# mbitsnbites/himg

Hardware: AMD Instinct MI355X
Metric: Mpixels/s encode+decode, 4K RGBA q=50 (higher is better)
Workload: dtype u8/i16/i32 integer

## Files before the change

himg_amd/__init__.py:

```python
import ctypes as C
import os

import numpy as np

from .build import LIB, build_lib

HIMG_OK = 0
HIMG_ERR_ARG = -1
HIMG_ERR_HIP = -2
HIMG_ERR_UNSUPPORTED = -3
HIMG_ERR_FORMAT = -4
HIMG_ERR_CAPACITY = -5
HIMG_ERR_TARGET = -6

HIMG_DT_F32 = 0
HIMG_DT_F16 = 1
HIMG_DT_BF16 = 2

SYNTH = {"grad": 0, "gradn": 1, "rand": 2, "randtile": 3}

DBG = {
    "avg": 0, "lowres": 1, "lres_sym": 2, "fres_sym": 3, "lres_hist": 4, "fres_hist": 5,
    "lres_len": 6, "fres_len": 7, "lres_code": 8, "fres_code": 9, "fres_row_bytes": 10,
    "dec_stats": 11, "parse_stats": 12, "rowcount_stats": 13, "loop_counts": 14, "fres_tok_sym": 15, "tok_cnt": 16,
}
DBG_DECODER = 0x100

_lib = None


class HimgError(RuntimeError):
    def __init__(self, code, msg=""):
        super().__init__("himg_hip error %d %s" % (code, msg))
        self.code = code


def lib():
    global _lib
    if _lib is not None:
        return _lib
    path = LIB
    if not os.path.exists(path):
        path = build_lib()
    try:
        import torch
    except ImportError:
        pass
    L = C.CDLL(path)
    vp, i32, u32, u64, sz = C.c_void_p, C.c_int, C.c_uint32, C.c_uint64, C.c_size_t
    P = C.POINTER
    L.himg_hip_create.argtypes = [i32, P(vp)]
    L.himg_hip_destroy.argtypes = [vp]
    L.himg_hip_destroy.restype = None
    L.himg_hip_last_error.argtypes = [vp]
    L.himg_hip_last_error.restype = C.c_char_p
    L.himg_hip_max_packed_size.argtypes = [i32, i32, i32]
    L.himg_hip_max_packed_size.restype = sz
    L.himg_hip_tok_layout.argtypes = [i32, i32, i32, i32, i32, i32, P(i32)]
    L.himg_hip_encode.argtypes = [vp, vp, i32, i32, i32, i32, i32, i32, P(vp), P(sz)]
    L.himg_hip_decode.argtypes = [vp, vp, sz, P(vp), P(i32), P(i32), P(i32)]
    L.himg_hip_encode_to.argtypes = [vp, vp, i32, i32, i32, i32, i32, i32, vp, sz, P(sz)]
    L.himg_hip_decode_to.argtypes = [vp, vp, sz, vp, sz, P(i32), P(i32), P(i32)]
    L.himg_hip_fetch_last.argtypes = [vp, vp, sz, P(sz)]
    L.himg_hip_peek.argtypes = [vp, sz, P(i32), P(i32), P(i32)]
    L.himg_hip_set_option.argtypes = [vp, i32, i32]
    L.himg_hip_get_option.argtypes = [vp, i32, C.POINTER(C.c_int)]
    L.himg_hip_encode_batch.argtypes = [vp, vp, i32, i32, i32, i32, i32, i32, i32, vp, vp, vp]
    L.himg_hip_decode_batch.argtypes = [vp, vp, vp, i32, vp, vp, vp, vp, vp]
    L.himg_hip_free.argtypes = [vp]
    L.himg_hip_free.restype = None
    L.himg_hip_host_alloc.argtypes = [sz]
    L.himg_hip_host_alloc.restype = vp
    L.himg_hip_host_free.argtypes = [vp]
    L.himg_hip_host_free.restype = None
    L.himg_hip_encode_device.argtypes = [vp, vp, i32, i32, i32, i32, i32, i32, i32, vp, sz, vp, vp, vp]
    L.himg_hip_decode_device.argtypes = [vp, vp, sz, vp, i32, i32, i32, i32, vp, vp, vp]
    L.himg_hip_encode_device_q.argtypes = [vp, vp, i32, i32, i32, i32, i32, vp, i32, vp, sz, vp, vp, vp]
    L.himg_hip_windows_extent.argtypes = [vp, i32, i32, vp, i32, i32, P(sz)]
    L.himg_hip_encode_windows_device.argtypes = [vp, vp, vp, i32, i32, vp, i32, i32, vp, i32, vp, sz, vp, vp, vp]
    L.himg_hip_encode_window_to.argtypes = [vp, vp, vp, i32, i32, i32, i32, i32, i32, i32, vp, sz, P(sz)]
    L.himg_hip_encode_sizes_device.argtypes = [vp, vp, i32, i32, i32, i32, i32, vp, i32, vp, vp, vp]
    L.himg_hip_budget_probes.argtypes = [i32, i32]
    L.himg_hip_encode_budget_device.argtypes = [vp, vp, i32, i32, i32, i32, i32, i32, i32, i32, vp, vp, sz, vp, vp, vp, vp]
    L.himg_hip_encode_budget_to.argtypes = [vp, vp, i32, i32, i32, i32, i32, i32, i32, sz, vp, sz, P(sz), P(i32)]
    L.himg_hip_encode_budget_batch.argtypes = [vp, vp, i32, i32, i32, i32, i32, i32, i32, i32, vp, vp, vp, vp, vp]
    L.himg_hip_encode_sse_device.argtypes = [vp, vp, i32, i32, i32, i32, i32, vp, i32, vp, vp, vp]
    L.himg_hip_encode_target_device.argtypes = [vp, vp, i32, i32, i32, i32, i32, i32, i32, i32, vp, vp, sz, vp, vp, vp, vp, vp]
    L.himg_hip_encode_target_to.argtypes = [vp, vp, i32, i32, i32, i32, i32, i32, i32, u64, vp, sz, P(sz), P(i32), P(u64)]
    L.himg_hip_encode_target_batch.argtypes = [vp, vp, i32, i32, i32, i32, i32, i32, i32, i32, vp, vp, vp, vp, vp, vp]
    L.himg_hip_psnr_to_sse.argtypes = [C.c_double, i32, i32, i32, P(u64)]
    L.himg_hip_decode_rows_device.argtypes = [vp, vp, C.c_uint32, i32, i32, i32, i32, i32, vp, vp, vp]
    L.himg_hip_decode_index_device.argtypes = [vp, vp, C.c_uint32, i32, i32, i32, vp, vp, vp, vp]
    L.himg_hip_decode_rows_indexed_device.argtypes = [vp, vp, C.c_uint32, i32, i32, i32, i32, i32, vp, vp, vp, vp]
    L.himg_hip_decode_rows_after_head_device.argtypes = [vp, vp, C.c_uint32, i32, i32, i32, i32, i32, vp, vp, vp, vp]
    L.himg_hip_decode_head_device.argtypes = [vp, vp, C.c_uint32, i32, i32, i32, vp]
    L.himg_hip_decode_first_device.argtypes = [vp, vp, C.c_uint32, i32, i32, i32, vp, vp, vp]
    L.himg_hip_decode_walk_device.argtypes = [vp, vp, C.c_uint32, i32, i32, i32, vp, vp, vp, vp]
    L.himg_hip_decode_walk_wait.argtypes = [vp]
    L.himg_hip_decode_walk_ranges_device.argtypes = [vp, vp, C.c_uint32, i32, i32, i32, C.POINTER(C.c_int), i32, vp, vp, vp, vp]
    L.himg_hip_decode_walk_wait_range.argtypes = [vp, i32]
    L.himg_hip_index_host.argtypes = [vp, sz, i32, P(i32), P(i32), P(i32), vp, sz, P(C.c_uint32)]
    L.himg_hip_preview_peek.argtypes = [vp, sz, sz, P(i32), P(i32), P(i32), P(sz)]
    L.himg_hip_region_peek.argtypes = [vp, sz, i32, i32, i32, i32, i32, vp]
    L.himg_hip_decode_region_to.argtypes = [vp, vp, sz, i32, i32, i32, i32, vp, sz, P(i32), P(i32), P(i32)]
    L.himg_hip_decode_region_device.argtypes = [vp, vp, sz, vp, i32, i32, i32, i32, i32, i32, i32, i32, vp, vp, vp]
    L.himg_hip_decode_regions_device.argtypes = [vp, vp, sz, vp, i32, i32, i32, i32, vp, i32, i32, vp, vp, vp]
    L.himg_hip_tensor_bytes.argtypes = [vp, i32, i32, i32, P(sz)]
    L.himg_hip_decode_tensor_device.argtypes = [vp, vp, sz, vp, i32, i32, i32, i32, vp, vp, vp, vp]
    L.himg_hip_decode_regions_tensor_device.argtypes = [vp, vp, sz, vp, i32, i32, i32, i32, vp, i32, i32, vp, vp, vp, vp]
    L.himg_hip_dst_extent.argtypes = [vp, i32, i32, vp, i32, i32, P(sz)]
    L.himg_hip_decode_into_device.argtypes = [vp, vp, sz, vp, i32, i32, i32, i32, vp, vp, vp, vp, vp]
    L.himg_hip_decode_regions_into_device.argtypes = [vp, vp, sz, vp, i32, i32, i32, i32, vp, i32, i32, vp, vp, vp, vp, vp]
    L.himg_hip_decode_into_to.argtypes = [vp, vp, sz, vp, vp, i32, i32, P(i32), P(i32), P(i32)]
    L.himg_hip_decode_regions_batch.argtypes = [vp, vp, vp, i32, vp, vp, vp, vp, vp, vp]
    L.himg_hip_scaled_size.argtypes = [i32, i32, i32, P(i32), P(i32)]
    L.himg_hip_decode_scaled_device.argtypes = [vp, vp, sz, vp, i32, i32, i32, i32, i32, vp, vp, vp]
    L.himg_hip_decode_scaled_to.argtypes = [vp, vp, sz, i32, vp, sz, P(i32), P(i32), P(i32)]
    L.himg_hip_decode_scaled_batch.argtypes = [vp, vp, vp, i32, i32, vp, vp, vp, vp, vp]
    L.himg_hip_pyramid_size.argtypes = [i32, i32, i32, P(i32), P(i32)]
    L.himg_hip_decode_pyramid_device.argtypes = [vp, vp, sz, vp, i32, i32, i32, i32, vp, vp, vp]
    L.himg_hip_decode_pyramid_to.argtypes = [vp, vp, sz, vp, vp, P(i32), P(i32), P(i32)]
    L.himg_hip_scaled_region_peek.argtypes = [vp, sz, i32, i32, i32, i32, i32, i32, vp]
    L.himg_hip_decode_scaled_region_to.argtypes = [vp, vp, sz, i32, i32, i32, i32, i32, vp, sz, P(i32), P(i32), P(i32)]
    L.himg_hip_decode_scaled_regions_device.argtypes = [vp, vp, sz, vp, i32, i32, i32, i32, i32, vp, i32, i32, vp, vp, vp]
    L.himg_hip_decode_scaled_regions_batch.argtypes = [vp, vp, vp, i32, i32, vp, vp, vp, vp, vp, vp]
    L.himg_hip_preview_to.argtypes = [vp, vp, sz, vp, sz, P(i32), P(i32), P(i32)]
    L.himg_hip_preview_batch.argtypes = [vp, vp, vp, i32, vp, vp, vp, vp, vp]
    L.himg_hip_preview_device.argtypes = [vp, vp, sz, vp, i32, i32, i32, i32, vp, vp, vp]
    L.himg_hip_prefix_peek.argtypes = [vp, sz, i32, vp]
    L.himg_hip_decode_prefix_to.argtypes = [vp, vp, sz, vp, sz, P(i32), P(i32), P(i32), P(i32)]
    L.himg_hip_decode_prefix_device.argtypes = [vp, vp, sz, vp, i32, i32, i32, i32, vp, vp, vp, vp]
    L.himg_hip_create_multi.argtypes = [vp, i32, P(vp)]
    L.himg_hip_destroy_multi.argtypes = [vp]
    L.himg_hip_destroy_multi.restype = None
    L.himg_hip_multi_count.argtypes = [vp]
    L.himg_hip_multi_last_error.argtypes = [vp]
    L.himg_hip_multi_last_error.restype = C.c_char_p
    L.himg_hip_multi_set_option.argtypes = [vp, i32, i32]
    L.himg_hip_multi_encode_batch.argtypes = [vp, vp, i32, i32, i32, i32, i32, i32, i32, vp, vp, vp]
    L.himg_hip_multi_decode_batch.argtypes = [vp, vp, vp, i32, vp, vp, vp, vp, vp]
    L.himg_hip_multi_encode.argtypes = [vp, vp, i32, i32, i32, i32, i32, i32, P(vp), P(sz)]
    L.himg_hip_multi_decode.argtypes = [vp, vp, sz, P(vp), P(i32), P(i32), P(i32)]
    L.himg_hip_shard_stats.argtypes = [vp, vp, i32, i32, i32, i32, i32, i32, i32, i32, vp, vp, vp]
    L.himg_hip_shard_row_bits.argtypes = [vp, vp, vp, vp]
    L.himg_hip_shard_emit.argtypes = [vp, vp, vp, sz, vp, vp]
    L.himg_hip_shard_assemble.argtypes = [vp, vp, vp, vp, sz, vp, sz, vp, vp, vp]
    L.himg_hip_shard_head.argtypes = [vp, vp, vp, vp, sz, vp, vp, vp, vp]
    L.himg_hip_shard_finish.argtypes = [vp, vp, sz, vp, vp]
    L.himg_hip_debug_read.argtypes = [vp, i32, i32, vp, sz, P(sz)]
    L.himg_hip_profile_enable.argtypes = [vp, i32]
    L.himg_hip_profile_reset.argtypes = [vp]
    L.himg_hip_profile_read.argtypes = [vp, P(i32), P(C.c_char_p), P(C.c_double), P(i32)]
    L.himg_synth_fill.argtypes = [i32, u64, i32, i32, vp]
    L.himg_fnv1a64.argtypes = [vp, sz]
    L.himg_fnv1a64.restype = u64
    L.himg_tables_shift.argtypes = [i32, i32, vp]
    L.himg_tables_shift.restype = None
    L.himg_tables_lowres_map.argtypes = [i32, vp]
    L.himg_tables_lowres_map.restype = None
    L.himg_tables_fullres_map.argtypes = [vp]
    L.himg_tables_fullres_map.restype = None
    L.himg_tables_map_to_8bit.argtypes = [vp, i32]
    L.himg_tables_map_to_8bit.restype = C.c_uint8
    _lib = L
    return L



def synth(kind, seed, width, height):
    a = np.empty((height, width, 4), np.uint8)
    rc = lib().himg_synth_fill(SYNTH[kind], seed, width, height, a.ctypes.data)
    if rc:
        raise HimgError(rc, "synth")
    return a


def fnv1a64(buf):
    b = np.ascontiguousarray(np.frombuffer(buf, np.uint8) if isinstance(buf, (bytes, bytearray)) else buf)
    return "%016x" % lib().himg_fnv1a64(b.ctypes.data, b.nbytes)


def max_packed_size(width, height, channels):
    return int(lib().himg_hip_max_packed_size(width, height, channels))


def budget_probes(qmin=0, qmax=100):
    n = lib().himg_hip_budget_probes(int(qmin), int(qmax))
    if n < 0:
        raise HimgError(n, "budget_probes")
    return n


def psnr_to_sse(psnr_db, width, height, channels):
    v = C.c_uint64()
    rc = lib().himg_hip_psnr_to_sse(float(psnr_db), int(width), int(height), int(channels), C.byref(v))
    if rc:
        raise HimgError(rc, "psnr_to_sse")
    return v.value


def tok_layout(width, height, channels=4, pixel_stride=None, row_tokens=-1, batch=1):
    out = (C.c_int32 * 6)()
    rc = lib().himg_hip_tok_layout(width, height, pixel_stride or channels, channels, row_tokens, batch, out)
    if rc != 0:
        raise ValueError("himg_hip_tok_layout: %d" % rc)
    return {"seg": out[0], "nseg": out[1], "cap": out[2], "stage_need": out[3], "stage": out[4], "tokens": bool(out[5])}


def pinned_empty(nbytes):
    import weakref
    ptr = lib().himg_hip_host_alloc(int(nbytes))
    if not ptr:
        raise MemoryError("himg_hip_host_alloc(%d)" % nbytes)
    buf = (C.c_uint8 * int(nbytes)).from_address(ptr)
    weakref.finalize(buf, lib().himg_hip_host_free, ptr)
    return np.frombuffer(buf, np.uint8)


def psnr(a, b):
    d = a.astype(np.float64) - b.astype(np.float64)
    mse = float(np.mean(d * d))
    return float("inf") if mse == 0 else 10.0 * np.log10(255.0 * 255.0 / mse)



_OPTIONS = {"fix_t2": 1, "count_wave": 2, "emit_rows": 3, "row_tokens": 4, "front": 5}


class Engine:

    def __init__(self, device=0):
        self._ctx = C.c_void_p()
        rc = lib().himg_hip_create(device, C.byref(self._ctx))
        if rc:
            raise HimgError(rc, "himg_hip_create (no usable GPU? there is no CPU fallback)")
        self.device = device
        self.fix_t2 = bool(self.get_option("fix_t2"))

    def close(self):
        if self._ctx:
            lib().himg_hip_destroy(self._ctx)
            self._ctx = C.c_void_p()

    def __del__(self):
        try:
            self.close()
        except Exception:
            pass

    def _check(self, rc, what):
        if rc:
            raise HimgError(rc, "%s: %s" % (what, lib().himg_hip_last_error(self._ctx).decode()))

    def _batch(self, fn, what, streams, outs, frame_bytes, *mid):
        n = len(streams)
        if outs is None:
            outs = [np.empty(max(frame_bytes(i, s_) or 0, 1), np.uint8) for i, s_ in enumerate(streams)]
        src = (C.c_void_p * n)(*[s_.ctypes.data for s_ in streams])
        szs = (C.c_size_t * n)(*[s_.nbytes for s_ in streams])
        dst = (C.c_void_p * n)(*[o.ctypes.data for o in outs])
        caps = (C.c_size_t * n)(*[o.nbytes for o in outs])
        ws, hs, cs = (C.c_int * n)(), (C.c_int * n)(), (C.c_int * n)()
        self._check(fn(self._ctx, src, szs, n, *mid, dst, caps, ws, hs, cs), what)
        return [o.ravel()[: ws[i] * hs[i] * cs[i]].reshape(hs[i], ws[i], cs[i]) for i, o in enumerate(outs)]

    def _encode_to(self, fn, what, img, channels, pixel_stride, mid, **results):
        img = np.ascontiguousarray(img, np.uint8)
        h, w, ch, stride = _image_geom(img, channels, pixel_stride)
        n = C.c_size_t()
        rc = fn(self._ctx, img.ctypes.data, w, h, stride, ch, *mid, None, 0, C.byref(n),
                *[C.byref(v) for v in results.values()])
        if rc != HIMG_ERR_CAPACITY or n.value == 0:
            e = HimgError(rc if rc != HIMG_OK else HIMG_ERR_ARG,
                          "%s: %s" % (what, lib().himg_hip_last_error(self._ctx).decode()))
            for name, v in results.items():
                setattr(e, name, v.value)
            raise e
        out = np.empty(n.value, np.uint8)
        self._check(lib().himg_hip_fetch_last(self._ctx, out.ctypes.data, out.nbytes, C.byref(n)), what)
        return (out, *[v.value for v in results.values()])

    def _encode_batch(self, fn, what, frames, outs, mid, results=(), soft=()):
        frames = [np.ascontiguousarray(f, np.uint8) for f in frames]
        n = len(frames)
        h, w, ch, stride = _image_geom(frames[0])
        if outs is None:
            outs = [np.empty(max_packed_size(w, h, ch), np.uint8) for _ in range(n)]
        src = (C.c_void_p * n)(*[f.ctypes.data for f in frames])
        dst = (C.c_void_p * n)(*[o.ctypes.data for o in outs])
        caps = (C.c_size_t * n)(*[o.nbytes for o in outs])
        sizes = (C.c_size_t * n)()
        rc = fn(self._ctx, src, n, w, h, stride, ch, *mid, dst, caps, sizes, *results)
        if rc not in (HIMG_OK, *soft):
            self._check(rc, what)
        return [o[: sizes[i]] for i, o in enumerate(outs)], rc

    def encode(self, img, quality=50, use_ycbcr=True, channels=None, pixel_stride=None):
        return self._encode_to(lib().himg_hip_encode_to, "encode", img, channels, pixel_stride,
                               (quality, 1 if use_ycbcr else 0))[0]

    def encode_window(self, data, src, x, y, w, h, quality=50, use_ycbcr=True, channels=None):
        data = _as_u8(data)
        ch = src.pixel_stride if channels is None else channels
        n = C.c_size_t()
        rc = lib().himg_hip_encode_window_to(self._ctx, data.ctypes.data, C.byref(src), ch, int(x), int(y), int(w),
                                             int(h), quality, 1 if use_ycbcr else 0, None, 0, C.byref(n))
        if rc != HIMG_ERR_CAPACITY or n.value == 0:
            self._check(rc if rc != HIMG_OK else HIMG_ERR_ARG, "encode_window")
        out = np.empty(n.value, np.uint8)
# ... 284 lines not shown
                                                         C.c_void_p(stream))
        self._check(rc, "decode_scaled_regions_device")

    def get_option(self, option):
        opt = _OPTIONS[option] if isinstance(option, str) else int(option)
        v = C.c_int(0)
        self._check(lib().himg_hip_get_option(self._ctx, opt, C.byref(v)), "get_option")
        return v.value

    def set_option(self, option, value):
        opt = _OPTIONS[option] if isinstance(option, str) else int(option)
        self._check(lib().himg_hip_set_option(self._ctx, opt, int(value)), "set_option")
        if opt == 1:
            self.fix_t2 = bool(value)

    def encode_device(self, d_frames, batch, width, height, pixel_stride, channels, quality,
                      use_ycbcr, d_out, out_stride, d_sizes, d_status, stream=0):
        rc = lib().himg_hip_encode_device(self._ctx, _ptr(d_frames), batch, width, height,
                                          pixel_stride, channels, quality, 1 if use_ycbcr else 0,
                                          _ptr(d_out), out_stride, _ptr(d_sizes), _ptr(d_status),
                                          C.c_void_p(stream))
        self._check(rc, "encode_device")

    def encode_device_q(self, d_frames, batch, width, height, pixel_stride, channels, qualities,
                        use_ycbcr, d_out, out_stride, d_sizes, d_status, stream=0):
        q = np.ascontiguousarray(np.asarray(qualities, np.int32).reshape(batch))
        rc = lib().himg_hip_encode_device_q(self._ctx, _ptr(d_frames), batch, width, height, pixel_stride, channels,
                                            q.ctypes.data, 1 if use_ycbcr else 0, _ptr(d_out), out_stride,
                                            _ptr(d_sizes), _ptr(d_status), C.c_void_p(stream))
        self._check(rc, "encode_device_q")

    def encode_windows_device(self, d_src, src, batch, channels, origins, w, h, qualities, use_ycbcr, d_out,
                              out_stride, d_sizes, d_status, stream=0):
        q = np.ascontiguousarray(np.asarray(qualities, np.int32).reshape(batch))
        org = np.ascontiguousarray(np.asarray(origins, np.int32).reshape(batch, 2))
        rc = lib().himg_hip_encode_windows_device(self._ctx, _ptr(d_src), C.byref(src), batch, channels,
                                                  org.ctypes.data, int(w), int(h), q.ctypes.data,
                                                  1 if use_ycbcr else 0, _ptr(d_out), out_stride, _ptr(d_sizes),
                                                  _ptr(d_status), C.c_void_p(stream))
        self._check(rc, "encode_windows_device")

    def encode_sizes_device(self, d_frames, batch, width, height, pixel_stride, channels, qualities,
                            use_ycbcr, d_sizes, d_status, stream=0):
        q = np.ascontiguousarray(np.asarray(qualities, np.int32).reshape(batch))
        rc = lib().himg_hip_encode_sizes_device(self._ctx, _ptr(d_frames), batch, width, height, pixel_stride,
                                                channels, q.ctypes.data, 1 if use_ycbcr else 0, _ptr(d_sizes),
                                                _ptr(d_status), C.c_void_p(stream))
        self._check(rc, "encode_sizes_device")

    def encode_budget_device(self, d_frames, batch, width, height, pixel_stride, channels, qmin, qmax,
                             use_ycbcr, budgets, d_out, out_stride, d_sizes, d_quality, d_status, stream=0):
        b = np.ascontiguousarray(np.minimum(np.asarray(budgets, np.uint64), 0xffffffff).astype(np.uint32).reshape(batch))
        rc = lib().himg_hip_encode_budget_device(self._ctx, _ptr(d_frames), batch, width, height, pixel_stride,
                                                 channels, int(qmin), int(qmax), 1 if use_ycbcr else 0,
                                                 b.ctypes.data, _ptr(d_out), out_stride, _ptr(d_sizes),
                                                 _ptr(d_quality), _ptr(d_status), C.c_void_p(stream))
        self._check(rc, "encode_budget_device")

    def encode_sse_device(self, d_frames, batch, width, height, pixel_stride, channels, qualities,
                          use_ycbcr, d_sse, d_status, stream=0):
        q = np.ascontiguousarray(np.asarray(qualities, np.int32).reshape(batch))
        rc = lib().himg_hip_encode_sse_device(self._ctx, _ptr(d_frames), batch, width, height, pixel_stride,
                                              channels, q.ctypes.data, 1 if use_ycbcr else 0, _ptr(d_sse),
                                              _ptr(d_status), C.c_void_p(stream))
        self._check(rc, "encode_sse_device")

    def encode_target_device(self, d_frames, batch, width, height, pixel_stride, channels, qmin, qmax,
                             use_ycbcr, max_sses, d_out, out_stride, d_sizes, d_quality, d_sse, d_status, stream=0):
        t = np.ascontiguousarray(np.array([min(max(int(x), 0), 2 ** 64 - 1) for x in max_sses], np.uint64).reshape(batch))
        rc = lib().himg_hip_encode_target_device(self._ctx, _ptr(d_frames), batch, width, height, pixel_stride,
                                                 channels, int(qmin), int(qmax), 1 if use_ycbcr else 0,
                                                 t.ctypes.data, _ptr(d_out), out_stride, _ptr(d_sizes),
                                                 _ptr(d_quality), _ptr(d_sse), _ptr(d_status), C.c_void_p(stream))
        self._check(rc, "encode_target_device")

    def decode_device(self, d_packed, in_stride, h_sizes, batch, width, height, channels, d_out,
                      d_status, stream=0):
        hs = np.ascontiguousarray(h_sizes, np.uint32)
        rc = lib().himg_hip_decode_device(self._ctx, _ptr(d_packed), in_stride, hs.ctypes.data,
                                          batch, width, height, channels, _ptr(d_out),
                                          _ptr(d_status), C.c_void_p(stream))
        self._check(rc, "decode_device")

    def decode_tensor_device(self, d_packed, in_stride, h_sizes, batch, width, height, channels, desc, d_out,
                             d_status, stream=0):
        hs = np.ascontiguousarray(h_sizes, np.uint32)
        rc = lib().himg_hip_decode_tensor_device(self._ctx, _ptr(d_packed), in_stride, hs.ctypes.data,
                                                 batch, width, height, channels, C.byref(desc), _ptr(d_out),
                                                 _ptr(d_status), C.c_void_p(stream))
        self._check(rc, "decode_tensor_device")

    def decode_rows_device(self, d_packed, packed_size, width, height, channels, row0, row1,
                           d_out_rows, d_status, stream=0):
        rc = lib().himg_hip_decode_rows_device(self._ctx, _ptr(d_packed), int(packed_size), width,
                                               height, channels, row0, row1, _ptr(d_out_rows),
                                               _ptr(d_status), C.c_void_p(stream))
        self._check(rc, "decode_rows_device")

    def decode_index_device(self, d_packed, packed_size, width, height, channels, d_row_index,
                            d_rows_first, d_status, stream=0):
        rc = lib().himg_hip_decode_index_device(self._ctx, _ptr(d_packed), int(packed_size), width, height,
                                                channels, _ptr(d_row_index), _ptr(d_rows_first),
                                                _ptr(d_status), C.c_void_p(stream))
        self._check(rc, "decode_index_device")

    def decode_rows_indexed_device(self, d_packed, packed_size, width, height, channels, row0, row1,
                                   d_row_index, d_out_rows, d_status, stream=0):
        rc = lib().himg_hip_decode_rows_indexed_device(self._ctx, _ptr(d_packed), int(packed_size), width,
                                                       height, channels, row0, row1, _ptr(d_row_index),
                                                       _ptr(d_out_rows), _ptr(d_status), C.c_void_p(stream))
        self._check(rc, "decode_rows_indexed_device")

    def decode_head_device(self, d_packed, packed_size, width, height, channels, stream=0):
        rc = lib().himg_hip_decode_head_device(self._ctx, _ptr(d_packed), int(packed_size), width, height,
                                               channels, C.c_void_p(stream))
        self._check(rc, "decode_head_device")

    def decode_rows_after_head_device(self, d_packed, packed_size, width, height, channels, row0, row1,
                                      d_row_index, d_out_rows, d_status, stream=0):
        rc = lib().himg_hip_decode_rows_after_head_device(self._ctx, _ptr(d_packed), int(packed_size), width,
                                                          height, channels, row0, row1, _ptr(d_row_index),
                                                          _ptr(d_out_rows), _ptr(d_status), C.c_void_p(stream))
        self._check(rc, "decode_rows_after_head_device")

    def decode_first_device(self, d_packed, packed_size, width, height, channels, d_rows_first, d_status,
                            stream=0):
        rc = lib().himg_hip_decode_first_device(self._ctx, _ptr(d_packed), int(packed_size), width, height,
                                                channels, _ptr(d_rows_first), _ptr(d_status), C.c_void_p(stream))
        self._check(rc, "decode_first_device")

    def decode_walk_device(self, d_packed, packed_size, width, height, channels, d_row_index, d_rows_first,
                           d_status, stream=0):
        rc = lib().himg_hip_decode_walk_device(self._ctx, _ptr(d_packed), int(packed_size), width, height, channels,
                                               _ptr(d_row_index), _ptr(d_rows_first), _ptr(d_status),
                                               C.c_void_p(stream))
        self._check(rc, "decode_walk_device")

    def decode_walk_ranges_device(self, d_packed, packed_size, width, height, channels, range_end, d_row_index,
                                  d_rows_first, d_range_status, stream=0):
        ends = (C.c_int * len(range_end))(*[int(x) for x in range_end])
        rc = lib().himg_hip_decode_walk_ranges_device(self._ctx, _ptr(d_packed), int(packed_size), width, height,
                                                      channels, ends, len(range_end), _ptr(d_row_index),
                                                      _ptr(d_rows_first), _ptr(d_range_status), C.c_void_p(stream))
        self._check(rc, "decode_walk_ranges_device")

    def decode_walk_wait_range(self, k):
        self._check(lib().himg_hip_decode_walk_wait_range(self._ctx, int(k)), "decode_walk_wait_range")

    def decode_walk_wait(self):
        self._check(lib().himg_hip_decode_walk_wait(self._ctx), "decode_walk_wait")

    def shard_stats(self, d_frame_base, width, height, pixel_stride, channels, quality, use_ycbcr,
                    row0, row1, d_hist, d_low_rows, stream=0):
        rc = lib().himg_hip_shard_stats(self._ctx, _ptr(d_frame_base), width, height, pixel_stride,
                                        channels, quality, 1 if use_ycbcr else 0, row0, row1,
                                        _ptr(d_hist), _ptr(d_low_rows), C.c_void_p(stream))
        self._check(rc, "shard_stats")

    def shard_row_bits(self, d_hist_global, d_row_bits, stream=0):
        rc = lib().himg_hip_shard_row_bits(self._ctx, _ptr(d_hist_global), _ptr(d_row_bits),
                                           C.c_void_p(stream))
        self._check(rc, "shard_row_bits")

    def shard_emit(self, d_all_row_bits, d_rel, rel_cap, d_rel_size, stream=0):
        rc = lib().himg_hip_shard_emit(self._ctx, _ptr(d_all_row_bits), _ptr(d_rel), rel_cap,
                                       _ptr(d_rel_size), C.c_void_p(stream))
# ... 357 lines not shown
```

himg_amd/csrc/dec_body_row_count_w.inc:

```
  __shared__ __attribute__((aligned(16))) uint32_t gyx[2 * kTabEntries];
  __shared__ uint32_t nd[kMaxNodes + 1];
  __shared__ __attribute__((aligned(16))) uint32_t s_stage[kCountRowsW * kStageAlloc];
  __shared__ int s_flag;
  uint32_t *gy = gyx, *gx = gyx + kTabEntries;
  const int f = blockIdx.y, tid = threadIdx.x, lane = tid & 63;
  DecFrame *df = ws.frames + f;
  if (tid == 0) {
    const int w = df->parse_status == 0 ? df->walk_status : 0;
    if (w && blockIdx.x == 0) atomicMax(&df->status, w);
    s_flag = df->status | w;
  }
  __syncthreads();
  const int failed = s_flag;
  if (!failed) {
    const uint32_t *nodes = ws.nodes + ((size_t)f * 2 + 1) * (kMaxNodes + 1);
    const int nn = df->s[1].num_nodes;
    for (int k = tid; k < nn; k += kDecThreads) nd[k] = nodes[k];
    const uint4 *gg = reinterpret_cast<const uint4 *>(ws.grp + ((size_t)f * 2 + 1) * (1u << kLutBits));
    for (int k = tid; k < (1 << kLutBits) / 2; k += kDecThreads) {
      const uint4 q = gg[k];
      reinterpret_cast<uint2 *>(gx)[k] = make_uint2(q.x, q.z);
      reinterpret_cast<uint2 *>(gy)[k] = make_uint2(q.y, q.w);
    }
    const uint4 *gs = reinterpret_cast<const uint4 *>(ws.sub + ((size_t)f * 2 + 1) * kSubEntries);
    for (int k = tid; k < kSubEntries / 2; k += kDecThreads) {
      const uint4 q = gs[k];
      reinterpret_cast<uint2 *>(gx + (1 << kLutBits))[k] = make_uint2(q.x, q.z);
      reinterpret_cast<uint2 *>(gy + (1 << kLutBits))[k] = make_uint2(q.y, q.w);
    }
  }
  __syncthreads();
  GrpTables tb;
  tb.grp = nullptr; tb.gx = gx; tb.gy = gy; tb.nd = nd;
  const int r = r0 + (int)blockIdx.x * kCountRowsW + (tid >> 6);
  if (r >= r1) return;
  const uint8_t *p = packed + (size_t)f * in_stride;
  uint32_t *l_start = ws.lane_start + ((size_t)f * g.rows + r) * kDecThreads;
  uint32_t *l_off = ws.lane_off + ((size_t)f * g.rows + r) * (kDecThreads + kRecHdr);
  if (lane == 0) l_off[kDecThreads + 2] = 0;
  const uint32_t pay_off = ws.row_off[(size_t)f * g.rows + r], pay_len = ws.row_len[(size_t)f * g.rows + r];
  const unsigned long long rem64 = 8ull * pay_len;
  uint32_t sb = (uint32_t)((rem64 + kDecThreads - 1) / kDecThreads);
  sb = (sb + 31u) & ~31u;
  sb = sb < kMinSubBits ? kMinSubBits : sb;
  if (failed || sb > (uint32_t)g.max_sub || rem64 == 0 || g.row_block >= (1 << 22)) return;
  const uint32_t rem = (uint32_t)rem64;
  GReader rd;
  const uint32_t rel0 = rd.attach(p, sizes[f], 8ull * pay_off);
  const uint32_t rel_end = rel0 + rem;
  const uint32_t lead = (uint32_t)g.lead_bits;
  uint32_t first = rel0;
  uint32_t base = 0;
  uint32_t rounds = 0;
  uint32_t *stage = s_stage + (tid >> 6) * kStageAlloc;
  LdsBits bits;
  bits.base = lds_addr(stage);
  auto phases = [&](auto staged_c) {
  constexpr bool STAGED = decltype(staged_c)::value;
#pragma unroll 1
  for (int j = 0; j < kDecThreads / 64; ++j) {
    const int v = 64 * j + lane;
    const SubGrid q = sub_grid(rel0, rem, sb, v);
    const bool active = q.active;
    const uint32_t pb0 = (uint32_t)__builtin_amdgcn_readfirstlane((int)q.b0);
    if (pb0 >= rel_end) {
      l_start[v] = rem;
      l_off[v] = base;
      continue;
    }
    uint32_t shift = 0;
    if constexpr (STAGED) {
      const uint32_t w0 = pb0 >> 5;
      shift = 32u * w0;
      wave_lds_sync();
      for (uint32_t k = (uint32_t)lane; 4u * k < kStageWords; k += 64u) {
        const uint32_t w = w0 + 4u * k;
        uint4 x;
        if (w + 3u <= rd.jmax) {
          const PackedU4 u = *reinterpret_cast<const PackedU4 *>(rd.w + w);
          x.x = u.x; x.y = u.y; x.z = u.z; x.w = u.w;
        } else {
          x.x = rd.ld(w); x.y = rd.ld(w + 1u); x.z = rd.ld(w + 2u); x.w = rd.ld(w + 3u);
        }
        uint32_t *d = stage + 4u * k + (k >> 3);
        d[0] = x.x; d[1] = x.y; d[2] = x.z; d[3] = x.w;
        if ((k & 7u) == 0u && k) d[-1] = x.x;
      }
      wave_lds_sync();
    }
    auto walk = [&](uint32_t from, uint32_t to, uint32_t *e, uint32_t *c, bool cont) {
      if constexpr (STAGED) { (void)cont; grp_count_lds(bits, tb, from, to, e, c); }
      else lean_count<true, GReader, true>(rd, tb, from, to, e, c, cont);
    };
    const uint32_t b0 = q.b0 - shift, lim = q.lim - shift, lo0 = rel0 - shift, fst = first - shift;
    uint32_t start = active ? b0 : rel_end - shift;
    if (lane == 0 && active) start = fst;
    bool at_start = false;
    if (lane > 0 && active && lead) {
      uint32_t from = start - lo0 > lead ? start - lead : lo0;
      if (from < pb0 - shift) from = pb0 - shift;
      uint32_t guess, none;
      walk(from, start, &guess, &none, false);
      start = guess;
      at_start = true;
    }
    uint32_t endpos = start, cnt = 0;
    bool dirty = active;
    uint32_t T = (active ? b0 : rel_end - shift) + kJoinBits;
    if (T > lim || T < b0) T = lim;
    uint32_t posT = ~0u, cT = 0;
    for (;;) {
      if (dirty) {
        uint32_t p1, c1;
        walk(start, T, &p1, &c1, at_start);
        if (p1 == posT) {
          cnt = c1 + (cnt - cT);
        } else {
          uint32_t c2;
          walk(p1, lim, &endpos, &c2, start < T || at_start);
          cnt = c1 + c2;
        }
        posT = p1;
        cT = c1;
        at_start = false;
      }
      const uint32_t ns = wave_shr1_dpp(fst, endpos);
      dirty = active && ns != start;
      if (active) start = ns;
      ++rounds;
      if (!__any(dirty ? 1 : 0)) break;
    }
    const uint32_t c = min(cnt, 0x3fffffu);
    const uint32_t incl = wave_scan_add_dpp(c);
    l_start[v] = start + shift - rel0;
    l_off[v] = base + incl - c;
    if (v == q.last_active) l_off[kDecThreads + 1] = endpos + shift - rel0;
    base += (uint32_t)__builtin_amdgcn_readlane((int)incl, 63);
    first = (uint32_t)__builtin_amdgcn_readlane((int)(active ? endpos + shift : rel_end), 63);
  }
  };
  if (sb <= kStageSubBits) phases(std::true_type{});
  else phases(std::false_type{});
  if (lane == 0) {
    l_off[kDecThreads] = base;
    l_off[kDecThreads + 3] = rounds;
    l_off[kDecThreads + 4] = 0;
    l_off[kDecThreads + 2] = 3;
  }
```

himg_amd/csrc/himg_dev.h:

```cpp
#ifndef HIMG_DEV_H_
#define HIMG_DEV_H_

#include <hip/hip_runtime.h>
#include <stdint.h>

#include "search_step.h"

namespace himg_dev {

constexpr int kNumSym = 261;
constexpr int kHistStride = 264;
constexpr int kLresSpan = 16384;
constexpr int kIterSyms = 4096;
constexpr int kTreeStride = 384;
constexpr int kMaxCodeLen = 32;
constexpr int kHeadLen = 175;

struct Geom {
  int W, H, C, stride;
  int rows, cols, mrows, mcols;
  int chan_size, lres_size;
  int row_block;
  int ycbcr;
  int lres_spans;
  int use_blocks;
  int fix_t2;
  int lres_serial;
  int max_sub;
  int lead_bits;
  int prefetch_rows;
  int count_wave;
  int wide_q;
  int emit_rows;
  int front;
  int row_tokens;
  long long frame_bytes;
  long long fres_size;
};

struct EncWs {
  uint8_t *avg, *low;        size_t plane_stride;
  uint8_t *lres_sym;         size_t lres_stride;
  uint8_t *fres_sym;         size_t fres_stride;
  uint32_t *hist;
  uint32_t *span_hist_l;
  uint32_t *span_hist_f;
  uint32_t *lres_trail;
  uint64_t *codes;
  uint32_t *lens;
  uint8_t *tree;
  uint32_t *tree_nbytes;
  uint64_t *span_bit0;
  uint32_t *span_bits;
  int32_t *status;
  uint16_t *tok;
  uint32_t *tok_cnt;
  int tok_seg, tok_nseg, tok_cap;
};

constexpr uint32_t kTokRunMark = 0x0100u;
constexpr int kTokMaxRun = 255;
constexpr int kTokIter = 2048;
constexpr int kTokRunPiece = 16662;
constexpr int kTokStage = 1152;
inline int tok_slots_beyond(int zeros_max) { return 5 + 3 * (zeros_max / kTokRunPiece); }
inline int tok_seg_pad(int row_block) {
  const int pad = (tok_slots_beyond(row_block) + 7) & ~7;
  return pad > 64 ? pad : 64;
}
inline int tok_stage_need(int row_block, int seg) {
  const int alone = 1024 + tok_slots_beyond(row_block);
  const int carried = 7 + 1024 + tok_slots_beyond(seg < row_block ? seg : row_block);
  return alone > carried ? alone : carried;
}

struct StaticChunks {
  uint8_t head[176];
  uint8_t mid[272];
  int mid_len;
};

struct ShiftTables {
  uint8_t s[2][64];
};

struct LresTables {
  int16_t tab[128];
  uint8_t code[512];
};

struct QualTab {
  uint32_t pq[3][2][64];
  ShiftTables st;
  LresTables lt;
  uint8_t lmap[128];
  uint8_t qcfg[64];
};
constexpr int kQualities = 101;
struct QualSel {
  const QualTab *tab;
  const int32_t *quality;
};

struct WinSrc {
  const uint8_t *base;
  size_t row_pitch, frame_pitch;
  const int32_t *org;
};


constexpr int kLutBits = 11;
constexpr int kDecThreads = 1024;
constexpr int kSubEntries = 1024;
constexpr int kSubMaxBits = 6;
// ... 80 lines not shown
                           const StaticChunks &sc, const QualSel &qs,
                           const uint8_t *d_fmap_lut, hipStream_t stream, Profiler *prof,
                           hipStream_t side, hipEvent_t ev_fork, hipEvent_t ev_join);
struct SearchState {
  int32_t *quality;
  uint64_t *limit, *best;
  uint64_t *value;
  int32_t *ok, *bad, *state, *err;
};
inline size_t search_state_bytes(int batch) { return ((((size_t)batch + 1) & ~(size_t)1) + 10 * (size_t)batch) * 4; }
inline SearchState search_state_carve(void *base, int batch) {
  const size_t b = (size_t)batch;
  int32_t *w = (int32_t *)base;
  uint64_t *d = (uint64_t *)(w + ((b + 1) & ~(size_t)1));
  int32_t *t = (int32_t *)(d + 3 * b);
  return SearchState{w, d, d + b, d + 2 * b, t, t + b, t + 2 * b, t + 3 * b};
}
void launch_search_step(const SearchState &ss, const EncWs &ws, int batch, int probe, int probes, int dir, int qmin,
                        int qmax, const uint32_t *d_sizes, int32_t *d_quality, hipStream_t stream, Profiler *prof);
void launch_search_finish(const SearchState &ss, const EncWs &ws, int batch, int miss_code, uint32_t *d_sizes,
                          uint64_t *d_sse, int32_t *d_status, hipStream_t stream, Profiler *prof);

struct SseTab {
  alignas(16) uint32_t w[128 + 32 + 64 + 4];
};
void sse_fill_tab(const int16_t fmap[128], const ShiftTables &st, SseTab *t);
struct SseArgs {
  uint8_t *rec;
  const SseTab *tab;
  uint64_t *sse;
};
void launch_sse(const Geom &g, const EncWs &ws, int batch, const uint8_t *d_frames, const QualSel &qs,
                const SseArgs &sa, hipStream_t stream, Profiler *prof);
void launch_encode_sse(const Geom &g, const EncWs &ws, int batch, const uint8_t *d_frames,
                       const StaticChunks &sc, const QualSel &qs, const SseArgs &sse,
                       const uint8_t *d_fmap_lut, hipStream_t stream, Profiler *prof,
                       hipStream_t side, hipEvent_t ev_fork, hipEvent_t ev_join);

constexpr int kWalkSegs = 4;
struct DecStreams {
  hipStream_t side = nullptr;
  hipStream_t side2 = nullptr;
  hipStream_t side3 = nullptr;
  hipEvent_t ev_fork = nullptr;
  hipEvent_t ev_walk[kWalkSegs] = {}, ev_cnt[kWalkSegs] = {}, ev_win[kWalkSegs] = {};
};

struct HostOpts {
  bool allow_fused = true;
  bool use_side = true;
  int walk_segs = 0;
  int persist_rows = 1;
  int n_cu = 256;
};

bool dec_rows_fit_lds(const Geom &g);
constexpr int kLoopCounters = 8;
int loop_counts_read_enc(unsigned long long *out);
int loop_counts_read_dec(unsigned long long *out);

struct TensDesc {
  int dtype, co;
  float scale[4], bias[4];
};
__host__ __device__ inline int tens_elem_size(int dtype) { return dtype == 0 ? 4 : 2; }

struct DstDesc {
  size_t row_pitch, frame_pitch;
  const int32_t *org;
  int pixel_stride;
};

struct PyrDesc {
  uint8_t *level[4];
};

void launch_decode(const Geom &g, const DecWs &ws, int batch, const uint8_t *d_packed,
                   size_t in_stride, const uint32_t *d_sizes, uint8_t *d_out,
                   int32_t *d_status, hipStream_t stream, Profiler *prof, const HostOpts &ho,
                   const DecStreams *ds, int r0, int r1,
                   const uint32_t *d_row_index = nullptr, bool index_only = false, int phase = 3,
                   const TensDesc *tens = nullptr, const DstDesc *dst = nullptr, const PyrDesc *pyr = nullptr);
constexpr int kDecHead = 1, kDecRows = 2;
void launch_preview(const Geom &g, const DecWs &ws, int batch, const uint8_t *d_packed, size_t in_stride,
                    const uint32_t *d_sizes, uint32_t *d_head_sizes, uint8_t *d_out, int32_t *d_status,
                    hipStream_t stream, Profiler *prof);
void launch_region(const Geom &g, const DecWs &ws, int batch, const uint8_t *d_packed, size_t in_stride,
                   const uint32_t *d_sizes, const uint32_t *d_row_index, const int32_t *h_org, const int32_t *d_org,
                   int scale_log2, int w, int h, uint8_t *d_out, int32_t *d_status, hipStream_t stream, Profiler *prof,
                   const DecStreams *ds, const TensDesc *tens = nullptr,
                   const DstDesc *dst = nullptr);
void launch_prefix(const Geom &g, const DecWs &ws, int batch, const uint8_t *d_packed, size_t in_stride,
                   uint32_t *d_words, uint8_t *d_out, int32_t *d_rows, int32_t *d_status, hipStream_t stream,
                   Profiler *prof, const DecStreams *ds);
int region_strip_tiles(const Geom &g);
void launch_scaled(const Geom &g, const DecWs &ws, int batch, const uint8_t *d_packed, size_t in_stride,
                   const uint32_t *d_sizes, const uint32_t *d_row_index, int scale_log2, uint8_t *d_out,
                   int32_t *d_status, hipStream_t stream, Profiler *prof, const DecStreams *ds);
int scaled_strip_tiles(const Geom &g, int scale_log2);
void launch_rowwalk_only(const Geom &g, const DecWs &ws, const uint8_t *d_packed, size_t in_stride,
                         const uint32_t *d_sizes, hipStream_t stream);
void launch_rowwalk_range(const Geom &g, const DecWs &ws, const uint8_t *d_packed, size_t in_stride,
                          const uint32_t *d_sizes, int row_end, bool resume, hipStream_t stream);

void launch_shard_stats(const Geom &g, const EncWs &ws, const uint8_t *d_frame_base,
                        const ShiftTables &st, const uint8_t *d_fmap_lut, int r0, int r1,
                        hipStream_t stream, Profiler *prof);
void launch_shard_row_bits(const Geom &g, const EncWs &ws, int r0, int r1, uint32_t *d_bits_out,
                           hipStream_t stream, Profiler *prof);
void launch_shard_emit(const Geom &g, const EncWs &ws, const StaticChunks &sc,
                       const uint32_t *d_all_row_bits, uint8_t *d_rel, size_t rel_cap,
                       uint32_t *d_rel_size, int r0, int r1, hipStream_t stream, Profiler *prof);
void launch_shard_assemble(const Geom &g, const EncWs &ws, const StaticChunks &sc,
                           const LresTables &lt, const uint32_t *d_all_row_bits,
                           const uint8_t *d_rel, size_t rel_bytes, uint8_t *d_out, size_t out_cap,
                           uint32_t *d_size, hipStream_t stream, Profiler *prof);

void launch_shard_head(const Geom &g, const EncWs &ws, const StaticChunks &sc, const LresTables &lt,
                       const uint32_t *d_all_row_bits, uint8_t *d_out, size_t out_cap, uint32_t *d_size,
                       uint32_t *d_head, int r0, int r1, hipStream_t stream, Profiler *prof);
void launch_shard_finish(const Geom &g, const EncWs &ws, uint8_t *d_out, size_t out_cap, const uint32_t *d_size,
                         hipStream_t stream, Profiler *prof);

hipError_t enc_set_kernel_attrs();
hipError_t dec_set_kernel_attrs();

void prof_begin(Profiler *p, const char *stage, hipStream_t s);
void prof_end(Profiler *p, hipStream_t s);

}
#endif
```

himg_amd/csrc/himg_hip.hip:

```cpp
#include "himg_hip.h"

#include <hip/hip_runtime.h>

#include <cmath>
#include <cstdio>
#include <cstdlib>
#include <cstring>
#include <string>
#include <vector>

#include "himg_dev.h"
#include "himg_tables.h"
#include "prefix_walk.h"

using namespace himg_dev;

namespace himg_dev {

struct Profiler {
  bool enabled = false;
  struct Rec { const char *name; hipEvent_t a, b; };
  std::vector<Rec> pending;
  struct Acc { std::string name; double ms = 0; int n = 0; };
  std::vector<Acc> acc;
// ... 2 lines not shown

  void collect() {
    for (auto &r : pending) {
      hipEventSynchronize(r.b);
      float ms = 0;
      hipEventElapsedTime(&ms, r.a, r.b);
      hipEventDestroy(r.a);
      hipEventDestroy(r.b);
      size_t i = 0;
      for (; i < acc.size(); ++i)
        if (acc[i].name == r.name) break;
      if (i == acc.size()) { acc.push_back(Acc()); acc.back().name = r.name; }
      acc[i].ms += ms;
      acc[i].n += 1;
    }
    pending.clear();
  }
};

void prof_begin(Profiler *p, const char *stage, hipStream_t s) {
  if (!p || !p->enabled) return;
  p->cur = stage;
  hipEventCreate(&p->cur_a);
  hipEventRecord(p->cur_a, s);
}
void prof_end(Profiler *p, hipStream_t s) {
  if (!p || !p->enabled) return;
  hipEvent_t b;
  hipEventCreate(&b);
  hipEventRecord(b, s);
  p->pending.push_back({p->cur, p->cur_a, b});
}

}

namespace {

struct DevBuf {
  void *p = nullptr;
  size_t cap = 0;
  bool reserve(size_t n) {
    if (n <= cap) return true;
    if (p) hipFree(p);
    p = nullptr;
    cap = 0;
    if (hipMalloc(&p, n) != hipSuccess) return false;
    cap = n;
    return true;
  }
  void release() {
    if (p) hipFree(p);
    p = nullptr;
    cap = 0;
  }
};

size_t round_up(size_t x, size_t a) { return (x + a - 1) / a * a; }

struct HostResult {
  uint32_t size;
  int32_t status;
  int32_t quality;
  uint64_t sse;
};
struct PipeMeta {
  HostResult res[2];
  uint32_t dec_size[2];
};

}

struct himg_hip_ctx {
  int device = 0;
  std::string err;
  Profiler prof;
  hipStream_t last_stream = nullptr;
  HostOpts opts;
  int fix_t2 = 0;
  int max_sub = 4096;
  int lead_bits = 128;
  int lres_serial = 0;
  int prefetch_rows = 1;
  int count_wave = -1, emit_rows = -1;
  int row_tokens = -1;
  int front = -1;
  DecStreams dstr;
  hipStream_t side_enc = nullptr;
  hipEvent_t ev_fork_e = nullptr, ev_join_e = nullptr;

  DevBuf fmap_lut;
  size_t host_bytes = 0;
  struct Pipe {
    bool ready = false;
    hipStream_t s_in = nullptr, s_comp = nullptr, s_out = nullptr;
    hipEvent_t ev_in[2] = {nullptr, nullptr}, ev_k[2] = {nullptr, nullptr}, ev_out[2] = {nullptr, nullptr};
    DevBuf in[2], out[2], meta[2];
    PipeMeta *h_meta = nullptr;
  } pipe;

  DevBuf e_planes, e_lres, e_fres, e_small, e_spanhist, e_tok, e_tokx;
  DevBuf e_qtab, e_search;
  DevBuf e_stab, e_rec;
  bool qtab_ready = false;
  Geom enc_geom{};
  EncWs enc_ws{};
  int enc_batch = 0;
  bool enc_valid = false;

  DevBuf d_frames, d_nodes, d_grp, d_gyc, d_sub, d_lane, d_rows, d_lres, d_fres, d_planes, d_sizes, d_stats, d_spec;
  Geom dec_geom{};
  DecWs dec_ws{};
  int dec_batch = 0;
  bool dec_valid = false;
  hipEvent_t ev_range[HIMG_MAX_WALK_RANGES] = {};
  int n_ranges = 0;
  struct HeadToken {
    bool valid = false;
    int w = 0, h = 0, c = 0;
    const void *packed = nullptr;
    uint32_t size = 0;
    void *stream = nullptr;
  } head;

  DevBuf h_in, h_out, h_result, h_status, h_index;
  uint32_t *hp_index = nullptr;
  size_t hp_index_cap = 0;

  struct SizeRing {
    static constexpr int kSlots = 4;
    uint32_t *h[kSlots] = {nullptr, nullptr, nullptr, nullptr};
    size_t cap[kSlots] = {0, 0, 0, 0};
    hipEvent_t ev[kSlots] = {nullptr, nullptr, nullptr, nullptr};
    bool busy[kSlots] = {false, false, false, false};
    int next = 0;
  } sizes_ring;

  struct {
    bool valid = false;
    Geom g{};
    StaticChunks sc{};
    ShiftTables st{};
    LresTables lt{};
    int r0 = 0, r1 = 0;
  } shard;
};

static int fail(himg_hip_ctx *ctx, int code, const char *what, hipError_t e = hipSuccess) {
  if (ctx) {
    ctx->err = what;
    if (e != hipSuccess) { ctx->err += ": "; ctx->err += hipGetErrorString(e); }
  }
  return code;
}

#define HIP_TRY(ctx, expr)                                                  \
  do {                                                                      \
    hipError_t e_ = (expr);                                                 \
    if (e_ != hipSuccess) return fail(ctx, HIMG_ERR_HIP, #expr, e_);        \
  } while (0)

static bool make_geom(int width, int height, int pixel_stride, int num_channels, int use_ycbcr,
                      Geom *g) {
  if (width < 1 || height < 1 || num_channels < 1 || num_channels > 4 ||
      pixel_stride < num_channels)
    return false;
  g->W = width; g->H = height; g->C = num_channels; g->stride = pixel_stride;
  g->rows = (height + 7) >> 3; g->cols = (width + 7) >> 3;
  g->mrows = (g->rows + 15) / 16; g->mcols = (g->cols + 15) / 16;
  g->chan_size = g->mrows * g->mcols + g->rows * g->cols;
  const long long lres = (long long)g->chan_size * num_channels;
  const long long fres = (long long)g->rows * g->cols * 64 * num_channels;
  if (fres > 0x7fffffffLL || (long long)width * height * pixel_stride > 0x7fffffffLL) return false;
  g->lres_size = (int)lres;
  g->row_block = g->cols * num_channels * 64;
  g->ycbcr = (use_ycbcr && num_channels >= 3) ? 1 : 0;
  g->lres_spans = (g->lres_size + kLresSpan - 1) / kLresSpan;
  g->use_blocks = g->rows > 1 ? 1 : 0;
  g->fix_t2 = 0;
  g->max_sub = 4096;
  g->lead_bits = 128;
  g->lres_serial = 0;
  g->count_wave = g->emit_rows = g->row_tokens = g->front = -1;
  g->wide_q = 0;
  g->prefetch_rows = 1;
  g->frame_bytes = (long long)width * height * pixel_stride;
  g->fres_size = fres;
  return true;
}

static void apply_settings(const himg_hip_ctx *ctx, Geom *g) {
  g->fix_t2 = ctx->fix_t2;
  g->max_sub = ctx->max_sub;
  g->lead_bits = ctx->lead_bits;
  g->lres_serial = ctx->lres_serial;
  g->prefetch_rows = ctx->prefetch_rows;
  g->count_wave = ctx->count_wave;
  g->emit_rows = ctx->emit_rows;
  g->row_tokens = ctx->row_tokens;
  g->front = ctx->front;
}

extern "C" size_t himg_hip_max_packed_size(int width, int height, int num_channels) {
  Geom g;
  if (!make_geom(width, height, num_channels, num_channels, 1, &g)) return 0;
  size_t n = 12 + 19 + 136 + 8 + 72 + 188 + 8;
  n += (size_t)g.lres_size + kTreeStride;
  n += (size_t)g.fres_size + kTreeStride + 4u * (size_t)g.rows;
  return round_up(n + 64, 256);
}

extern "C" int himg_hip_create(int device, himg_hip_ctx **out) {
  if (!out) return HIMG_ERR_ARG;
  *out = nullptr;
  int count = 0;
  if (hipGetDeviceCount(&count) != hipSuccess || count < 1) return HIMG_ERR_HIP;
  if (device < 0 || device >= count) return HIMG_ERR_ARG;
  if (hipSetDevice(device) != hipSuccess) return HIMG_ERR_HIP;
  himg_hip_ctx *ctx = new himg_hip_ctx();
  ctx->device = device;
  HostOpts &o = ctx->opts;
  if (const char *e = std::getenv("HIMG_FORCE_UNFUSED")) o.allow_fused = !(e[0] == '1');
  if (const char *e = std::getenv("HIMG_WALK_SEGS")) o.walk_segs = atoi(e);
  if (const char *e = std::getenv("HIMG_SIDE_STREAM")) o.use_side = !(e[0] == '0');
  if (const char *e = std::getenv("HIMG_PERSIST_ROWS")) o.persist_rows = atoi(e);
  if (const char *e = std::getenv("HIMG_PREFETCH_ROWS")) ctx->prefetch_rows = atoi(e);
  if (const char *e = std::getenv("HIMG_FIX_T2")) ctx->fix_t2 = e[0] == '1';
  if (const char *e = std::getenv("HIMG_FORCE_LRES_SERIAL")) ctx->lres_serial = e[0] == '1';
  if (const char *e = std::getenv("HIMG_MAX_SUB_BITS")) {
    const int v = std::atoi(e);
    if (v >= 128 && v <= 4096 && v % 32 == 0) ctx->max_sub = v;
  }
  if (const char *e = std::getenv("HIMG_COUNT_WAVE")) ctx->count_wave = atoi(e) ? 1 : 0;
  if (const char *e = std::getenv("HIMG_EMIT_ROWS")) ctx->emit_rows = atoi(e) ? 1 : 0;
  if (const char *e = std::getenv("HIMG_ROW_TOKENS")) ctx->row_tokens = atoi(e) ? 1 : 0;
  if (const char *e = std::getenv("HIMG_FRONT")) ctx->front = atoi(e) ? 1 : 0;
  if (const char *e = std::getenv("HIMG_LEAD_BITS")) {
    const int v = std::atoi(e);
    if (v >= 0 && v <= 4096) ctx->lead_bits = v;
  }
  int n_cu = 0;
  if (hipDeviceGetAttribute(&n_cu, hipDeviceAttributeMultiprocessorCount, device) == hipSuccess && n_cu > 0) o.n_cu = n_cu;
  if (himg_dev::enc_set_kernel_attrs() != hipSuccess || himg_dev::dec_set_kernel_attrs() != hipSuccess) {
    delete ctx;
    return HIMG_ERR_HIP;
  }
  std::vector<uint8_t> lut(32769);
  int16_t fmap[128];
  himg_tables_fullres_map(fmap);
  for (int a = 0; a <= 32767; ++a) lut[a] = himg_tables_map_to_8bit(fmap, a);
  lut[32768] = (uint8_t)(0u - himg_tables_map_to_8bit(fmap, -32768));
  if (!ctx->fmap_lut.reserve(round_up(lut.size(), 256)) ||
      hipMemcpy(ctx->fmap_lut.p, lut.data(), lut.size(), hipMemcpyHostToDevice) != hipSuccess) {
    delete ctx;
    return HIMG_ERR_HIP;
  }
  int prio_least = 0, prio_greatest = 0;
  (void)hipDeviceGetStreamPriorityRange(&prio_least, &prio_greatest);
  bool ev_ok = true;
  for (int k = 0; k < kWalkSegs; ++k)
    ev_ok = ev_ok && hipEventCreateWithFlags(&ctx->dstr.ev_walk[k], hipEventDisableTiming) == hipSuccess &&
            hipEventCreateWithFlags(&ctx->dstr.ev_cnt[k], hipEventDisableTiming) == hipSuccess &&
            hipEventCreateWithFlags(&ctx->dstr.ev_win[k], hipEventDisableTiming) == hipSuccess;
  if (!ev_ok || hipStreamCreateWithPriority(&ctx->dstr.side, hipStreamNonBlocking, prio_least) != hipSuccess ||
      hipStreamCreateWithPriority(&ctx->dstr.side2, hipStreamNonBlocking, prio_least) != hipSuccess ||
      hipEventCreateWithFlags(&ctx->dstr.ev_fork, hipEventDisableTiming) != hipSuccess ||
      hipStreamCreateWithFlags(&ctx->side_enc, hipStreamNonBlocking) != hipSuccess ||
      hipEventCreateWithFlags(&ctx->ev_fork_e, hipEventDisableTiming) != hipSuccess ||
      hipEventCreateWithFlags(&ctx->ev_join_e, hipEventDisableTiming) != hipSuccess) {
    himg_hip_destroy(ctx);
    return HIMG_ERR_HIP;
  }
  ctx->dstr.side3 = ctx->side_enc;
  *out = ctx;
  return HIMG_OK;
}

extern "C" void himg_hip_destroy(himg_hip_ctx *ctx) {
  if (!ctx) return;
  hipSetDevice(ctx->device);
  hipDeviceSynchronize();
  if (ctx->dstr.ev_fork) hipEventDestroy(ctx->dstr.ev_fork);
  for (int k = 0; k < kWalkSegs; ++k) {
    if (ctx->dstr.ev_walk[k]) hipEventDestroy(ctx->dstr.ev_walk[k]);
    if (ctx->dstr.ev_cnt[k]) hipEventDestroy(ctx->dstr.ev_cnt[k]);
    if (ctx->dstr.ev_win[k]) hipEventDestroy(ctx->dstr.ev_win[k]);
  }
  for (int k = 0; k < HIMG_MAX_WALK_RANGES; ++k)
    if (ctx->ev_range[k]) hipEventDestroy(ctx->ev_range[k]);
  if (ctx->dstr.side) hipStreamDestroy(ctx->dstr.side);
  if (ctx->dstr.side2) hipStreamDestroy(ctx->dstr.side2);
  if (ctx->ev_fork_e) hipEventDestroy(ctx->ev_fork_e);
  if (ctx->ev_join_e) hipEventDestroy(ctx->ev_join_e);
  if (ctx->side_enc) hipStreamDestroy(ctx->side_enc);
  for (int k = 0; k < himg_hip_ctx::SizeRing::kSlots; ++k) {
    if (ctx->sizes_ring.ev[k]) hipEventDestroy(ctx->sizes_ring.ev[k]);
    if (ctx->sizes_ring.h[k]) hipHostFree(ctx->sizes_ring.h[k]);
  }
  ctx->prof.collect();
  if (ctx->pipe.ready) {
    for (int k = 0; k < 2; ++k) {
      hipEventDestroy(ctx->pipe.ev_in[k]); hipEventDestroy(ctx->pipe.ev_k[k]); hipEventDestroy(ctx->pipe.ev_out[k]);
      ctx->pipe.in[k].release(); ctx->pipe.out[k].release(); ctx->pipe.meta[k].release();
    }
    hipStreamDestroy(ctx->pipe.s_in); hipStreamDestroy(ctx->pipe.s_comp); hipStreamDestroy(ctx->pipe.s_out);
    hipHostFree(ctx->pipe.h_meta);
  }
  DevBuf *all[] = {&ctx->fmap_lut, &ctx->e_planes, &ctx->e_lres, &ctx->e_fres, &ctx->e_small,
                   &ctx->e_spanhist, &ctx->e_tok, &ctx->e_tokx, &ctx->e_qtab, &ctx->e_search, &ctx->e_stab, &ctx->e_rec, &ctx->d_frames, &ctx->d_nodes, &ctx->d_grp, &ctx->d_gyc, &ctx->d_sub, &ctx->d_lane, &ctx->d_rows,
                   &ctx->d_lres, &ctx->d_fres, &ctx->d_planes, &ctx->d_sizes, &ctx->d_stats, &ctx->d_spec, &ctx->h_in,
                   &ctx->h_out, &ctx->h_result, &ctx->h_status, &ctx->h_index};
  for (DevBuf *b : all) b->release();
  if (ctx->hp_index) hipHostFree(ctx->hp_index);
  delete ctx;
}

extern "C" const char *himg_hip_last_error(const himg_hip_ctx *ctx) {
  return ctx ? ctx->err.c_str() : "no context";
}

extern "C" void himg_hip_free(void *p) { std::free(p); }

extern "C" void *himg_hip_host_alloc(size_t bytes) {
  void *p = nullptr;
  if (hipHostMalloc(&p, bytes ? bytes : 1, hipHostMallocDefault) != hipSuccess) return nullptr;
  return p;
}
extern "C" void himg_hip_host_free(void *p) {
  if (p) (void)hipHostFree(p);
}

extern "C" int himg_hip_get_option(himg_hip_ctx *ctx, int option, int *value) {
  if (!ctx || !value) return HIMG_ERR_ARG;
  if (option == HIMG_OPT_FIX_T2) { *value = ctx->fix_t2; return HIMG_OK; }
  if (option == HIMG_OPT_COUNT_WAVE) { *value = ctx->count_wave; return HIMG_OK; }
  if (option == HIMG_OPT_EMIT_ROWS) { *value = ctx->emit_rows; return HIMG_OK; }
  if (option == HIMG_OPT_ROW_TOKENS) { *value = ctx->row_tokens; return HIMG_OK; }
  if (option == HIMG_OPT_FRONT) { *value = ctx->front; return HIMG_OK; }
  return fail(ctx, HIMG_ERR_ARG, "unknown option");
}

extern "C" int himg_hip_set_option(himg_hip_ctx *ctx, int option, int value) {
  if (!ctx) return HIMG_ERR_ARG;
  if (option == HIMG_OPT_FIX_T2) { ctx->fix_t2 = value ? 1 : 0; return HIMG_OK; }
  const int tri = value < 0 ? -1 : (value ? 1 : 0);
  if (option == HIMG_OPT_COUNT_WAVE) { ctx->count_wave = tri; return HIMG_OK; }
  if (option == HIMG_OPT_EMIT_ROWS) { ctx->emit_rows = tri; return HIMG_OK; }
  if (option == HIMG_OPT_FRONT) { ctx->front = tri; return HIMG_OK; }
  if (option == HIMG_OPT_ROW_TOKENS) { ctx->row_tokens = value == 2 ? 2 : tri; return HIMG_OK; }
  return fail(ctx, HIMG_ERR_ARG, "unknown option");
}

static void put_u32(uint8_t *p, uint32_t x) {
  p[0] = (uint8_t)x; p[1] = (uint8_t)(x >> 8); p[2] = (uint8_t)(x >> 16); p[3] = (uint8_t)(x >> 24);
}

static int build_static(const Geom &g, int quality, StaticChunks *sc, ShiftTables *st,
                        LresTables *lt) {
  memset(sc, 0, sizeof(*sc));
  uint8_t *h = sc->head;
  memcpy(h, "RIFF", 4); put_u32(h + 4, 0); memcpy(h + 8, "HIMG", 4);
  memcpy(h + 12, "FRMT", 4); put_u32(h + 16, 11);
  h[20] = 1; put_u32(h + 21, (uint32_t)g.W); put_u32(h + 25, (uint32_t)g.H);
  h[29] = (uint8_t)g.C; h[30] = (uint8_t)g.ycbcr;
  int16_t lmap[128], fmap[128];
  himg_tables_lowres_map(quality, lmap);
  memcpy(h + 31, "LMAP", 4);
  const int ln = himg_tables_mapping_function(lmap, h + 39);
  if (ln != 128) return HIMG_ERR_UNSUPPORTED;
  put_u32(h + 35, (uint32_t)ln);
  memcpy(h + 167, "LRES", 4);
  himg_tables_shift(quality, 0, st->s[0]);
  himg_tables_shift(quality, 1, st->s[1]);
  uint8_t *m = sc->mid;
  int o = 0;
  memcpy(m + o, "QCFG", 4); put_u32(m + o + 4, g.ycbcr ? 64u : 32u); o += 8;
  for (int t = 0; t < (g.ycbcr ? 2 : 1); ++t)
    for (int i = 0; i < 32; ++i) m[o++] = (uint8_t)((st->s[t][2 * i] << 4) | st->s[t][2 * i + 1]);
  himg_tables_fullres_map(fmap);
  memcpy(m + o, "FMAP", 4);
  const int fn = himg_tables_mapping_function(fmap, m + o + 8);
  put_u32(m + o + 4, (uint32_t)fn);
  o += 8 + fn;
  memcpy(m + o, "FRES", 4); o += 8;
  sc->mid_len = o;
  memcpy(lt->tab, lmap, sizeof(lmap));
  for (int d = -255; d <= 255; ++d) lt->code[d + 255] = himg_tables_map_to_8bit(lmap, d);
  lt->code[511] = 0;
  return HIMG_OK;
}

extern "C" int himg_hip_tok_layout(int width, int height, int pixel_stride, int num_channels, int row_tokens,
                                   int batch, int out[6]) {
  Geom g;
  if (!out || batch < 1 || !make_geom(width, height, pixel_stride, num_channels, 1, &g)) return HIMG_ERR_ARG;
  g.row_tokens = row_tokens;
  const int seg = himg_dev::enc_tok_seg(g);
  out[0] = seg;
  out[1] = (g.row_block + seg - 1) / seg;
  out[2] = seg + himg_dev::tok_seg_pad(g.row_block);
  out[3] = himg_dev::tok_stage_need(g.row_block, seg);
  out[4] = himg_dev::kTokStage;
  out[5] = himg_dev::enc_uses_row_tokens(g, batch) ? 1 : 0;
  return HIMG_OK;
}

static int stage_words(himg_hip_ctx *ctx, void *d_dst, const void *a, size_t na, const void *b, size_t nb, hipStream_t s) {
  auto &r = ctx->sizes_ring;
  const int k = r.next;
  r.next = (k + 1) % himg_hip_ctx::SizeRing::kSlots;
  if (!r.ev[k]) HIP_TRY(ctx, hipEventCreateWithFlags(&r.ev[k], hipEventDisableTiming));
  if (r.busy[k]) HIP_TRY(ctx, hipEventSynchronize(r.ev[k]));
  const size_t words = na + nb;
  if (r.cap[k] < words) {
    if (r.h[k]) hipHostFree(r.h[k]);
    r.h[k] = nullptr;
    r.cap[k] = 0;
    const size_t want = words < 64 ? 64 : words;
    HIP_TRY(ctx, hipHostMalloc((void **)&r.h[k], want * 4, hipHostMallocDefault));
    r.cap[k] = want;
  }
  memcpy(r.h[k], a, na * 4);
  if (nb) memcpy(r.h[k] + na, b, nb * 4);
  HIP_TRY(ctx, hipMemcpyAsync(d_dst, r.h[k], words * 4, hipMemcpyHostToDevice, s));
  HIP_TRY(ctx, hipEventRecord(r.ev[k], s));
  r.busy[k] = true;
  return HIMG_OK;
// ... 462 lines not shown
  if (probes < 0) return fail(ctx, HIMG_ERR_ARG, "the quality range must satisfy 0 <= qmin <= qmax <= 100");
  if (!h_limits || !d_sizes || !d_quality || (k.probe_sse && (!k.d_sse || ((uintptr_t)k.d_sse & 7))))
    return fail(ctx, HIMG_ERR_ARG, "bad argument");
  Enc e;
  int rc = enc_q_begin(ctx, d_frames, batch, width, height, pixel_stride, num_channels, use_ycbcr, true, d_out, out_stride,
                       k.probe_sse, stream, &e);
  if (rc) return rc;
  const size_t lim_at = (size_t)((int32_t *)e.ss.limit - e.ss.quality);
  std::vector<int32_t> w0(lim_at + 2 * (size_t)batch, k.dir == himg_dev::kSearchFromMin ? qmin : qmax);
  for (int i = 0; i < batch; ++i) {
    const uint64_t lim = h_limits[i];
    memcpy(w0.data() + lim_at + 2 * (size_t)i, &lim, 8);
  }
  if ((rc = stage_words(ctx, e.ss.quality, w0.data(), w0.size(), nullptr, 0, e.s))) return rc;
  for (int p = 0; p < probes; ++p) {
    if (k.probe_sse) sse_launch(ctx, e, batch, d_frames, e.ss.value);
    else enc_q_launch(ctx, e, batch, d_frames, nullptr, 0, d_sizes);
    himg_dev::launch_search_step(e.ss, ctx->enc_ws, batch, p, probes, k.dir, qmin, qmax, k.probe_sse ? nullptr : d_sizes,
                                 d_quality, e.s, &ctx->prof);
  }
  enc_q_launch(ctx, e, batch, d_frames, d_out, out_stride, d_sizes);
  himg_dev::launch_search_finish(e.ss, ctx->enc_ws, batch, k.miss_code, d_sizes, k.d_sse, d_status, e.s, &ctx->prof);
  return enc_end(ctx, e, batch, nullptr);
}

extern "C" int himg_hip_encode_budget_device(himg_hip_ctx *ctx, const void *d_frames, int batch, int width, int height,
                                             int pixel_stride, int num_channels, int qmin, int qmax, int use_ycbcr,
                                             const uint32_t *h_budgets, void *d_out, size_t out_stride,
                                             uint32_t *d_sizes, int32_t *d_quality, int32_t *d_status, void *stream) {
  const EncSearch k = {himg_dev::kSearchFromMin, false, HIMG_ERR_CAPACITY, nullptr};
  return encode_search_device(ctx, k, d_frames, batch, width, height, pixel_stride, num_channels, qmin, qmax, use_ycbcr,
                              h_budgets, d_out, out_stride, d_sizes, d_quality, d_status, stream);
}

extern "C" int himg_hip_encode_target_device(himg_hip_ctx *ctx, const void *d_frames, int batch, int width, int height,
                                             int pixel_stride, int num_channels, int qmin, int qmax, int use_ycbcr,
                                             const uint64_t *h_max_sse, void *d_out, size_t out_stride,
                                             uint32_t *d_sizes, int32_t *d_quality, uint64_t *d_sse, int32_t *d_status,
                                             void *stream) {
  const EncSearch k = {himg_dev::kSearchFromMax, true, HIMG_ERR_TARGET, d_sse};
  return encode_search_device(ctx, k, d_frames, batch, width, height, pixel_stride, num_channels, qmin, qmax, use_ycbcr,
                              h_max_sse, d_out, out_stride, d_sizes, d_quality, d_status, stream);
}

extern "C" int himg_hip_psnr_to_sse(double psnr_db, int width, int height, int num_channels, uint64_t *max_sse) {
  Geom g;
  if (!max_sse || !std::isfinite(psnr_db) || psnr_db < 0.0 ||
      !make_geom(width, height, num_channels, num_channels, 1, &g))
    return HIMG_ERR_ARG;
  const double n = (double)width * (double)height * (double)num_channels;
  *max_sse = (uint64_t)floor(255.0 * 255.0 * n / pow(10.0, psnr_db / 10.0));
  return HIMG_OK;
}

static int decode_full(himg_hip_ctx *ctx, const void *d_packed, size_t in_stride, const uint32_t *h_sizes, int batch,
                       int width, int height, int num_channels, void *d_out, int32_t *d_status, void *stream,
                       const char *bad, const himg_dev::TensDesc *td, himg_dev::DstDesc *dd, const int32_t *h_org,
                       const himg_dev::PyrDesc *pm = nullptr) {
  Geom g;
  const uint32_t *d_sizes = nullptr;
  if (int rc = decode_args(ctx, width, height, num_channels, batch, kWsFull, d_packed, d_out, &in_stride, bad, &g))
    return rc;
  if (int rc = stride_covers(ctx, h_sizes, batch, in_stride)) return rc;
  { uint32_t mx = 0; for (int i = 0; i < batch; ++i) mx = h_sizes[i] > mx ? h_sizes[i] : mx; g.wide_q = wide_q_hint(g, mx); }
  if (int rc = decode_begin(ctx, g, batch, kWsFull, h_sizes, stream, &d_sizes, dd ? h_org : nullptr)) return rc;
  if (dd) dd->org = (const int32_t *)(d_sizes + batch);
  launch_decode(g, ctx->dec_ws, batch, (const uint8_t *)d_packed, in_stride, d_sizes, (uint8_t *)d_out, d_status,
                (hipStream_t)stream, &ctx->prof, ctx->opts, ctx->opts.use_side ? &ctx->dstr : nullptr, 0, g.rows,
                nullptr, false, 3, td, dd, pm);
  HIP_TRY(ctx, hipGetLastError());
  return HIMG_OK;
}

extern "C" int himg_hip_decode_device(himg_hip_ctx *ctx, const void *d_packed, size_t in_stride,
                                      const uint32_t *h_sizes, int batch, int width, int height,
                                      int num_channels, void *d_out, int32_t *d_status,
                                      void *stream) {
  if (!ctx || !d_packed || !h_sizes || !d_out || !d_status || batch < 1 || batch > 65535)
    return HIMG_ERR_ARG;
  return decode_full(ctx, d_packed, in_stride, h_sizes, batch, width, height, num_channels, d_out, d_status, stream,
                     nullptr, nullptr, nullptr, nullptr);
}

static bool tensor_desc_ok(const himg_hip_tensor_desc *t, int C, himg_dev::TensDesc *td) {
  if (!t || t->dtype < HIMG_DT_F32 || t->dtype > HIMG_DT_BF16 || t->out_channels < 1 || t->out_channels > C || C > 4)
    return false;
  himg_dev::TensDesc d = {};
  d.dtype = t->dtype; d.co = t->out_channels;
  for (int c = 0; c < t->out_channels; ++c) {
    if (!std::isfinite(t->scale[c]) || !std::isfinite(t->bias[c])) return false;
    d.scale[c] = t->scale[c]; d.bias[c] = t->bias[c];
  }
  if (td) *td = d;
  return true;
}

extern "C" int himg_hip_tensor_bytes(const himg_hip_tensor_desc *t, int num_channels, int w, int h,
                                     size_t *bytes_per_frame) {
  Geom g;
  if (!bytes_per_frame || !make_geom(w, h, num_channels, num_channels, 1, &g) || !tensor_desc_ok(t, num_channels, nullptr))
    return HIMG_ERR_ARG;
  *bytes_per_frame = (size_t)t->out_channels * (size_t)h * (size_t)w * (size_t)himg_dev::tens_elem_size(t->dtype);
  return HIMG_OK;
}

extern "C" int himg_hip_decode_tensor_device(himg_hip_ctx *ctx, const void *d_packed, size_t in_stride,
                                             const uint32_t *h_sizes, int batch, int width, int height,
                                             int num_channels, const himg_hip_tensor_desc *t, void *d_out,
                                             int32_t *d_status, void *stream) {
  if (!ctx || !d_packed || !h_sizes || !t || !d_out || !d_status || batch < 1 || batch > 65535)
    return HIMG_ERR_ARG;
  himg_dev::TensDesc td;
  const char *bad = tensor_desc_ok(t, num_channels, &td) ? nullptr : "bad tensor descriptor";
  return decode_full(ctx, d_packed, in_stride, h_sizes, batch, width, height, num_channels, d_out, d_status, stream, bad,
                     &td, nullptr, nullptr);
}

static const char *dst_check(const himg_hip_dst *dst, int num_channels, int batch, const int32_t *h_origins, int w, int h,
                             size_t *bytes, himg_dev::DstDesc *dd = nullptr) {
  if (!dst) return "bad argument";
  const himg_hip_src s = {dst->width, dst->height, dst->pixel_stride, dst->row_pitch, dst->frame_pitch};
  if (const char *bad = windows_check(&s, num_channels, batch, h_origins, w, h, bytes)) return bad;
  if (dd) { dd->row_pitch = dst->row_pitch; dd->frame_pitch = dst->frame_pitch; dd->org = nullptr; dd->pixel_stride = dst->pixel_stride; }
  return nullptr;
}

extern "C" int himg_hip_dst_extent(const himg_hip_dst *dst, int num_channels, int batch, const int32_t *h_origins,
                                   int w, int h, size_t *bytes) {
  if (!bytes) return HIMG_ERR_ARG;
  *bytes = 0;
  return dst_check(dst, num_channels, batch, h_origins, w, h, bytes) ? HIMG_ERR_ARG : HIMG_OK;
}

extern "C" int himg_hip_decode_into_device(himg_hip_ctx *ctx, const void *d_packed, size_t in_stride,
                                           const uint32_t *h_sizes, int batch, int width, int height,
                                           int num_channels, void *d_dst, const himg_hip_dst *dst,
                                           const int32_t *h_origins, int32_t *d_status, void *stream) {
  if (!ctx || !d_packed || !h_sizes || !d_dst || !d_status || batch < 1 || batch > 65535) return HIMG_ERR_ARG;
  himg_dev::DstDesc dd;
  size_t extent = 0;
  const char *bad = dst_check(dst, num_channels, batch, h_origins, width, height, &extent, &dd);
  return decode_full(ctx, d_packed, in_stride, h_sizes, batch, width, height, num_channels, d_dst, d_status, stream, bad,
                     nullptr, &dd, h_origins);
}

extern "C" int himg_hip_decode_rows_device(himg_hip_ctx *ctx, const void *d_packed, uint32_t packed_size,
                                           int width, int height, int num_channels, int row0,
                                           int row1, void *d_out_rows, int32_t *d_status,
                                           void *stream) {
  if (!ctx || !d_packed || !d_out_rows || !d_status) return HIMG_ERR_ARG;
  Geom g;
  const uint32_t *d_sizes = nullptr;
  if (int rc = decode_args(ctx, width, height, num_channels, 1, kWsFull, d_packed, d_out_rows, nullptr,
                           bad_row_range(height, row0, row1), &g))
    return rc;
  g.wide_q = wide_q_hint(g, packed_size);
  if (int rc = decode_begin(ctx, g, 1, kWsFull, &packed_size, stream, &d_sizes)) return rc;
  uint8_t *base = (uint8_t *)d_out_rows - (size_t)8 * row0 * g.W * g.C;
  launch_decode(g, ctx->dec_ws, 1, (const uint8_t *)d_packed, ((size_t)packed_size + 3) / 4 * 4, d_sizes, base, d_status,
                (hipStream_t)stream, &ctx->prof, ctx->opts, ctx->opts.use_side ? &ctx->dstr : nullptr, row0, row1);
  HIP_TRY(ctx, hipGetLastError());
  return HIMG_OK;
}

extern "C" int himg_hip_decode_index_device(himg_hip_ctx *ctx, const void *d_packed, uint32_t packed_size,
                                            int width, int height, int num_channels,
// ... 1564 lines not shown
                              hipMemcpyDeviceToDevice, s));
  launch_shard_head(sh.g, ctx->enc_ws, sh.sc, sh.lt, d_all_row_bits, (uint8_t *)d_out, out_cap, d_size, d_head,
                    sh.r0, sh.r1, s, &ctx->prof);
  if (d_status)
    hipLaunchKernelGGL(k_copy_status, dim3(1), dim3(64), 0, s, ctx->enc_ws.status, d_status, 1);
  HIP_TRY(ctx, hipGetLastError());
  return HIMG_OK;
}

extern "C" int himg_hip_shard_finish(himg_hip_ctx *ctx, void *d_out, size_t out_cap, const uint32_t *d_size,
                                     void *stream) {
  if (!ctx || !ctx->shard.valid || !d_out || !d_size) return HIMG_ERR_ARG;
  HIP_TRY(ctx, hipSetDevice(ctx->device));
  launch_shard_finish(ctx->shard.g, ctx->enc_ws, (uint8_t *)d_out, out_cap, d_size, (hipStream_t)stream, &ctx->prof);
  HIP_TRY(ctx, hipGetLastError());
  return HIMG_OK;
}

extern "C" int himg_hip_debug_read(himg_hip_ctx *ctx, int what, int frame, void *dst,
                                   size_t dst_bytes, size_t *written) {
  if (!ctx || !dst) return HIMG_ERR_ARG;
  HIP_TRY(ctx, hipSetDevice(ctx->device));
  HIP_TRY(ctx, hipDeviceSynchronize());
  const void *src = nullptr;
  size_t n = 0;
  const bool dec = (what & 0x100) != 0;
  what &= 0xff;
  if (what == HIMG_DBG_LOOP_COUNTS) {
    unsigned long long c[2 * himg_dev::kLoopCounters];
    if (dst_bytes < sizeof(c)) return HIMG_ERR_CAPACITY;
    if ((dec ? himg_dev::loop_counts_read_dec(c) : himg_dev::loop_counts_read_enc(c)) != 0) return HIMG_ERR_ARG;
    memcpy(dst, c, sizeof(c));
    if (written) *written = sizeof(c);
    return HIMG_OK;
  }
  if (!dec) {
    if (!ctx->enc_valid || frame < 0 || frame >= ctx->enc_batch) return HIMG_ERR_ARG;
    const Geom &g = ctx->enc_geom;
    const EncWs &w = ctx->enc_ws;
    const int nsp = g.lres_spans + g.rows;
    switch (what) {
      case HIMG_DBG_AVG: src = w.avg + frame * w.plane_stride; n = (size_t)g.C * g.rows * g.cols; break;
      case HIMG_DBG_LOWRES: src = w.low + frame * w.plane_stride; n = (size_t)g.C * g.rows * g.cols; break;
      case HIMG_DBG_LRES_SYM: src = w.lres_sym + frame * w.lres_stride; n = (size_t)g.lres_size; break;
      case HIMG_DBG_FRES_SYM: src = w.fres_sym + frame * w.fres_stride; n = (size_t)g.fres_size; break;
      case HIMG_DBG_FRES_TOK_SYM: {
        if (!w.tok) return HIMG_ERR_ARG;
        if (!ctx->e_tokx.reserve(round_up((size_t)g.fres_size + 16, 256))) return fail(ctx, HIMG_ERR_HIP, "scratch plane allocation failed");
        himg_dev::launch_tok_expand(g, w, frame, (uint8_t *)ctx->e_tokx.p, nullptr);
        HIP_TRY(ctx, hipDeviceSynchronize());
        src = ctx->e_tokx.p; n = (size_t)g.fres_size; break;
      }
      case HIMG_DBG_TOK_CNT:
        if (!w.tok) return HIMG_ERR_ARG;
        src = w.tok_cnt + (size_t)frame * g.rows * w.tok_nseg; n = (size_t)g.rows * w.tok_nseg * 4; break;
      case HIMG_DBG_LRES_HIST: src = w.hist + ((size_t)frame * 2 + 0) * kHistStride; n = kNumSym * 4; break;
      case HIMG_DBG_FRES_HIST: src = w.hist + ((size_t)frame * 2 + 1) * kHistStride; n = kNumSym * 4; break;
      case HIMG_DBG_LRES_LEN: src = w.lens + ((size_t)frame * 2 + 0) * kHistStride; n = kNumSym * 4; break;
      case HIMG_DBG_FRES_LEN: src = w.lens + ((size_t)frame * 2 + 1) * kHistStride; n = kNumSym * 4; break;
      case HIMG_DBG_LRES_CODE: src = w.codes + ((size_t)frame * 2 + 0) * kHistStride; n = kNumSym * 8; break;
      case HIMG_DBG_FRES_CODE: src = w.codes + ((size_t)frame * 2 + 1) * kHistStride; n = kNumSym * 8; break;
      case HIMG_DBG_FRES_ROW_BYTES: {
        std::vector<uint32_t> bits(g.rows);
        HIP_TRY(ctx, hipMemcpy(bits.data(), w.span_bits + (size_t)frame * nsp + g.lres_spans,
                               (size_t)g.rows * 4, hipMemcpyDeviceToHost));
        n = (size_t)g.rows * 4;
        if (dst_bytes < n) return HIMG_ERR_CAPACITY;
        for (int r = 0; r < g.rows; ++r) ((uint32_t *)dst)[r] = (bits[r] + 7) >> 3;
        if (written) *written = n;
        return HIMG_OK;
      }
      default: return HIMG_ERR_ARG;
    }
  } else {
    if (!ctx->dec_valid || frame < 0 || frame >= ctx->dec_batch) return HIMG_ERR_ARG;
    const Geom &g = ctx->dec_geom;
    const DecWs &w = ctx->dec_ws;
    switch (what) {
      case HIMG_DBG_LOWRES: src = w.low + frame * w.plane_stride; n = (size_t)g.C * g.rows * g.cols; break;
      case HIMG_DBG_LRES_SYM: src = w.lres_sym + frame * w.lres_stride; n = (size_t)g.lres_size; break;
      case HIMG_DBG_FRES_SYM: src = w.fres_sym ? w.fres_sym + frame * w.fres_stride : nullptr; n = (size_t)g.fres_size; break;
      case HIMG_DBG_DEC_STATS: src = w.stats + (size_t)frame * (g.rows + 1) * 8; n = (size_t)(g.rows + 1) * 32; break;
      case HIMG_DBG_PARSE_STATS: src = w.parse_stats + (size_t)frame * 4; n = 16; break;
      case HIMG_DBG_ROWCOUNT_STATS: src = w.rc_stats ? w.rc_stats + (size_t)frame * g.rows * 8 : nullptr; n = (size_t)g.rows * 32; break;
      default: return HIMG_ERR_ARG;
    }
    if (!src) return HIMG_ERR_ARG;
  }
  if (dst_bytes < n) return HIMG_ERR_CAPACITY;
  HIP_TRY(ctx, hipMemcpy(dst, src, n, hipMemcpyDeviceToHost));
  if (written) *written = n;
  return HIMG_OK;
}

extern "C" int himg_hip_profile_enable(himg_hip_ctx *ctx, int enable) {
  if (!ctx) return HIMG_ERR_ARG;
  ctx->prof.enabled = enable != 0;
  return HIMG_OK;
}

extern "C" int himg_hip_profile_reset(himg_hip_ctx *ctx) {
  if (!ctx) return HIMG_ERR_ARG;
  hipSetDevice(ctx->device);
  ctx->prof.collect();
  ctx->prof.acc.clear();
  return HIMG_OK;
}

extern "C" int himg_hip_profile_read(himg_hip_ctx *ctx, int *n_stages,
                                     const char *names[HIMG_MAX_STAGES],
                                     double ms[HIMG_MAX_STAGES], int launches[HIMG_MAX_STAGES]) {
  if (!ctx || !n_stages) return HIMG_ERR_ARG;
  hipSetDevice(ctx->device);
  ctx->prof.collect();
  int n = 0;
  for (auto &a : ctx->prof.acc) {
    if (n >= HIMG_MAX_STAGES) break;
    names[n] = a.name.c_str();
    ms[n] = a.ms;
    launches[n] = a.n;
    ++n;
  }
  *n_stages = n;
  return HIMG_OK;
}
```

himg_amd/csrc/kernels_dec.hip:

```cpp
#include "himg_dev.h"
#include "prefix_walk.h"
#include "loop_counts.h"

#include <cstdlib>
#include <type_traits>

namespace himg_dev {

__device__ static constexpr uint8_t kScanD[64] = {
    0,  1,  9,  8,  16, 17, 18, 10, 2,  3,  11, 19, 27, 26, 25, 24,
    32, 33, 34, 35, 36, 28, 20, 12, 4,  5,  13, 21, 29, 37, 45, 44,
    43, 42, 41, 40, 48, 49, 50, 51, 52, 53, 54, 46, 38, 30, 22, 14,
    6,  7,  15, 23, 31, 39, 47, 55, 63, 62, 61, 60, 59, 58, 57, 56};

__device__ static constexpr uint8_t kInvScanD[64] = {
    0, 1, 8, 9, 24, 25, 48, 49, 3, 2, 7, 10, 23, 26, 47, 50, 4, 5, 6, 11, 22, 27, 46, 51, 15, 14, 13, 12, 21, 28, 45, 52, 16, 17, 18, 19, 20, 29, 44, 53, 35, 34, 33, 32, 31, 30, 43, 54, 36, 37, 38, 39, 40, 41, 42, 55, 63, 62, 61, 60, 59, 58, 57, 56};

constexpr int kStGeom = 1, kStUnsupported = 3, kStFormat = 4;
__device__ __host__ constexpr int fmt_err(int stage, int huff) { return kStFormat | (stage << 4) | (huff << 8); }
constexpr int kMaxDepth = 32;
constexpr int kMaxNodes = 2 * kNumSym - 1;
constexpr int kMaxSlow = 128;

__device__ __forceinline__ int clamp255d(int x) { return x < 0 ? 0 : (x > 255 ? 255 : x); }
// ... 2839 lines not shown
    lean_fixpoint<true, RD, 0, 3>(rd, tb, sh, rel0, active, lim, &start, &endpos, &cnt, &rounds, false, lead_bits, nullptr,
                                  c_phase, nullptr, mark, mcnt);
  } else {
    lean_fixpoint<true>(rd, tb, sh, rel0, active, lim, &start, &endpos, &cnt, &rounds, false, lead_bits, nullptr, c_phase);
  }
  const long long c_fix1 = clock64();
  uint32_t tot;
  const uint32_t cc = min(cnt, 0x3fffffu);
  const uint32_t off = block_scan_u32d(cc, sm32, &tot);
  l_start[tid] = start - rel0;
  l_off[tid] = off;
  if (QTR) {
    uint32_t o[5];
    o[0] = off; o[4] = off + cc;
#pragma unroll
    for (int k = 0; k < 3; ++k) {
      o[k + 1] = off + min(mcnt[k], cc);
      l_q[k * kDecThreads + tid] = mark[k] - rel0;
      l_q[(3 + k) * kDecThreads + tid] = o[k + 1];
    }
    if (window && cc) {
      for (uint32_t w = (o[0] + window - 1u) / window; w * window < o[4] && w * window < out_size && w < (uint32_t)(kRecHdr - kRecWin); ++w) {
        if (w == 0) continue;
        const uint32_t X = w * window;
        int k = 0;
#pragma unroll
        for (int j = 1; j < 4; ++j) if (X >= o[j]) k = j;
        l_off[kDecThreads + kRecWin + w] = 4u * (uint32_t)tid + (uint32_t)k;
      }
    }
  }
  if (tid == last_active) l_off[kDecThreads + 1] = endpos - rel0;
  if (tid == 0) {
    l_off[kDecThreads] = tot;
    l_off[kDecThreads + 3] = rounds | (min(sh->dbg[0], 4095u) << 8) | (min(sh->dbg[1], 4095u) << 20);
    l_off[kDecThreads + 4] = QTR ? 1u : 0u;
    l_off[kDecThreads + 2] = 1;
  }
  if ((tid & 63) == 0 && rc) {
    atomicMax(&rc[0], (uint32_t)((c_fix0 - c_in) >> 4));
    atomicMax(&rc[1], (uint32_t)(c_phase[0] >> 4));
    atomicMax(&rc[2], (uint32_t)(c_phase[1] >> 4));
    atomicMax(&rc[3], (uint32_t)((c_fix1 - c_fix0) >> 4));
    atomicMax(&rc[4], (uint32_t)((clock64() - c_in) >> 4));
  }
}

template <bool LDSPAY>
__global__ __launch_bounds__(kDecThreads, 8) void k_row_count(Geom g, DecWs ws, const uint8_t *packed,
                                                           size_t in_stride, const uint32_t *sizes,
                                                           int r0, int r1, int rows_per_wg) {
#include "dec_body_row_count.inc"
}

constexpr int kCountRowsW = kDecThreads / 64;

template <int CTRL, int ROW_MASK>
__device__ __forceinline__ uint32_t dpp_from_d(uint32_t identity, uint32_t v) {
  return (uint32_t)__builtin_amdgcn_update_dpp((int)identity, (int)v, CTRL, ROW_MASK, 0xf, false);
}
__device__ __forceinline__ uint32_t wave_scan_add_dpp(uint32_t v) {
  v += dpp_from_d<0x111, 0xf>(0, v);
  v += dpp_from_d<0x112, 0xf>(0, v);
  v += dpp_from_d<0x114, 0xf>(0, v);
  v += dpp_from_d<0x118, 0xf>(0, v);
  v += dpp_from_d<0x142, 0xa>(0, v);
  v += dpp_from_d<0x143, 0xc>(0, v);
  return v;
}
__device__ __forceinline__ uint32_t wave_shr1_dpp(uint32_t first, uint32_t v) {
  return dpp_from_d<0x138, 0xf>(first, v);
}

typedef u32x2 u32x2_a4 __attribute__((aligned(4)));
struct LdsBits {
  uint32_t base;
  __device__ __forceinline__ uint32_t window(uint32_t pos) const {
    const uint32_t w = pos >> 5;
    const uint32_t a = base + ((w + (w >> 5)) << 2);
    const u32x2 x = *(const __attribute__((address_space(3))) u32x2_a4 *)(uintptr_t)a;
    return __builtin_amdgcn_alignbit(x.y, x.x, pos);
  }
};
constexpr uint32_t kStageSubBits = 320;
constexpr uint32_t kStageWords = 64u * kStageSubBits / 32u + 32u;
constexpr uint32_t kStageAlloc = (kStageWords + kStageWords / 32u + 3u) & ~3u;
static_assert(kStageWords % 32 == 0, "whole blocks");

struct BitWin64 {
  unsigned long long win;
  __device__ __forceinline__ void consume(int n) { win >>= n; }
  __device__ __forceinline__ void refill() {}
};

__device__ __forceinline__ void grp_count_lds(const LdsBits &bits, const GrpTables &t, uint32_t pos, uint32_t lim,
                                              uint32_t *endpos, uint32_t *count) {
  uint32_t c = 0;
  if (pos < lim) {
    bool bad = false;
    const uint32_t TM = (uint32_t)kLutBits;
    const uint32_t TB = lds_addr(t.gy);
    const uint32_t XOFF = (uint32_t)kTabEntries * 4u;
    uint32_t tm = TM, tb = TB;
    auto step = [&]() {
      uint32_t win = bits.window(pos);
      uint32_t a;
      asm("v_lshl_add_u32 %0, %1, 2, %2" : "=v"(a) : "v"(__builtin_amdgcn_ubfe(win, 0u, tm)), "v"(tb));
      uint32_t y = lds_ld32(a);
      uint32_t ntm = TM, ntb = TB;
      if (__builtin_expect(y == 0, 0)) {
        const uint32_t x = lds_ld32(a + XOFF);
        if ((x >> 31) && tm == TM) {
          ntm = x & 255u;
          ntb = TB + (((1u << kLutBits) + ((x >> 8) & 0xffffu)) << 2);
          y = (uint32_t)kLutBits | ((uint32_t)kLutBits << 27);
        } else {
          BitWin64 rd;
          rd.win = (unsigned long long)win | ((unsigned long long)bits.window(pos + 32u) << 32);
          const int base = tm == TM ? 0 : kLutBits;
          uint32_t len, by;
          y = walk_token(rd, t, x, base, &len, &by, &bad);
          pos += len - (uint32_t)base;
          win = bits.window(pos);
        }
      }
      tm = ntm; tb = ntb;
      const uint32_t extra = __builtin_amdgcn_ubfe(win, y, y >> 5);
      pos += y >> 27;
      c += ((y >> 10) & 511u) + extra;
    };
    LoopCount lc;
    while (pos < lim) { HIMG_REGION_BEGIN("dec.count"); step(); lc.step(); HIMG_REGION_END("dec.count"); }
    lc.done(1);
    if (tm != TM) step();
  }
  *endpos = pos;
  *count = c;
}

__global__ __launch_bounds__(kDecThreads, 8) void k_row_count_w(Geom g, DecWs ws, const uint8_t *packed,
                                                               size_t in_stride, const uint32_t *sizes,
                                                               int r0, int r1) {
#include "dec_body_row_count_w.inc"
}

constexpr int kQPhases = 4;
__device__ __forceinline__ uint32_t *qrec_pos(uint32_t *l_start, uint32_t *l_q, uint32_t q) {
  const uint32_t t = q >> 2, k = q & 3u;
  return k == 0 ? l_start + t : l_q + (k - 1u) * kDecThreads + t;
}
__device__ __forceinline__ uint32_t *qrec_off(uint32_t *l_off, uint32_t *l_q, uint32_t q) {
  const uint32_t t = q >> 2, k = q & 3u;
  return k == 0 ? l_off + t : l_q + (2u + k) * kDecThreads + t;
}
__global__ __launch_bounds__(kDecThreads, 8) void k_row_count_q(Geom g, DecWs ws, const uint8_t *packed,
                                                               size_t in_stride, const uint32_t *sizes, int r0) {
  __shared__ __attribute__((aligned(16))) uint32_t gyx[2 * kTabEntries];
  __shared__ uint32_t nd[kMaxNodes + 1];
  __shared__ __attribute__((aligned(16))) uint32_t s_stage[kCountRowsW * kStageAlloc];
  __shared__ int s_flag;
  __shared__ uint32_t s_ws[kCountRowsW], s_we[kCountRowsW], s_wc[kCountRowsW], s_wl[kCountRowsW], s_bad;
  uint32_t *gy = gyx, *gx = gyx + kTabEntries;
  const int f = blockIdx.y, r = r0 + (int)blockIdx.x, tid = threadIdx.x, lane = tid & 63, wave = tid >> 6;
  DecFrame *df = ws.frames + f;
  if (tid == 0) {
    const int w = df->parse_status == 0 ? df->walk_status : 0;
    if (w && blockIdx.x == 0) atomicMax(&df->status, w);
    s_flag = df->status | w;
  }
  __syncthreads();
  const int failed = s_flag;
  const size_t ri = (size_t)f * g.rows + (size_t)r;
  uint32_t *l_start = ws.lane_start + ri * kDecThreads;
  uint32_t *l_off = ws.lane_off + ri * (kDecThreads + kRecHdr);
  uint32_t *l_q = ws.lane_q + ri * (6 * kDecThreads);
  if (tid == 0) l_off[kDecThreads + 2] = 0;
  if (tid >= kRecWin && tid < kRecHdr) l_off[kDecThreads + tid] = ~0u;
  const uint32_t pay_off = ws.row_off[ri], pay_len = ws.row_len[ri];
  const unsigned long long rem64 = 8ull * pay_len;
  uint32_t sb1 = (uint32_t)((rem64 + kDecThreads - 1) / kDecThreads);
  sb1 = (sb1 + 31u) & ~31u;
  sb1 = sb1 < kMinSubBits ? kMinSubBits : sb1;
  constexpr uint32_t NSUB = 4u * (uint32_t)kDecThreads;
  uint32_t sb = (uint32_t)((rem64 + NSUB - 1u) / NSUB);
  sb = (sb + 31u) & ~31u;
  sb = sb < kMinSubBits ? kMinSubBits : sb;
  if (failed || sb1 > (uint32_t)g.max_sub || rem64 == 0 || g.row_block >= (1 << 22) || sb > kStageSubBits) return;
  {
    const uint32_t *nodes = ws.nodes + ((size_t)f * 2 + 1) * (kMaxNodes + 1);
    const int nn = df->s[1].num_nodes;
    for (int k = tid; k < nn; k += kDecThreads) nd[k] = nodes[k];
    const uint4 *gg = reinterpret_cast<const uint4 *>(ws.grp + ((size_t)f * 2 + 1) * (1u << kLutBits));
    for (int k = tid; k < (1 << kLutBits) / 2; k += kDecThreads) {
      const uint4 q = gg[k];
      reinterpret_cast<uint2 *>(gx)[k] = make_uint2(q.x, q.z);
      reinterpret_cast<uint2 *>(gy)[k] = make_uint2(q.y, q.w);
    }
    const uint4 *gs = reinterpret_cast<const uint4 *>(ws.sub + ((size_t)f * 2 + 1) * kSubEntries);
    for (int k = tid; k < kSubEntries / 2; k += kDecThreads) {
      const uint4 q = gs[k];
      reinterpret_cast<uint2 *>(gx + (1 << kLutBits))[k] = make_uint2(q.x, q.z);
      reinterpret_cast<uint2 *>(gy + (1 << kLutBits))[k] = make_uint2(q.y, q.w);
    }
  }
  __syncthreads();
  GrpTables tb;
  tb.grp = nullptr; tb.gx = gx; tb.gy = gy; tb.nd = nd;
  const uint32_t rem = (uint32_t)rem64;
  GReader rd;
  const uint32_t rel0 = rd.attach(packed + (size_t)f * in_stride, sizes[f], 8ull * pay_off);
  const uint32_t rel_end = rel0 + rem;
  const uint32_t lead = (uint32_t)g.lead_bits;
  uint32_t *stage = s_stage + wave * kStageAlloc;
  LdsBits bits;
  bits.base = lds_addr(stage);
  uint32_t w_start = rel_end, w_end = rel_end, w_last = rel_end, w_cnt = 0, rounds = 0;
  auto run_wave = [&](uint32_t first0, bool exact0) {
    uint32_t first = first0, base = 0;
    bool have_start = false;
#pragma unroll 1
    for (int j = 0; j < kQPhases; ++j) {
      const uint32_t v = 256u * (uint32_t)wave + 64u * (uint32_t)j + (uint32_t)lane;
      const uint32_t nb0 = v ? rel0 + v * sb : rel0;
      uint32_t nlim = rel0 + (v + 1u) * sb;
      if (nlim > rel_end) nlim = rel_end;
      const bool active = nb0 < rel_end;
      const uint32_t pb0 = (uint32_t)__builtin_amdgcn_readfirstlane((int)nb0);
// ... 486 lines not shown
#include "dec_body_region.inc"
}

struct RegionArgsT {
  Geom g;
  DecWs ws;
  const uint8_t *packed;
  size_t in_stride;
  const uint32_t *sizes;
  RegionArgs ra;
  TensDesc t;
};
__global__ __launch_bounds__(kDecThreads) void k_dec_region_t(RegionArgsT a) {
  constexpr bool kRegionTens = true, kRegionPitch = false;
  const DstK pd = nullptr;
  const Geom &g = a.g;
  const DecWs &ws = a.ws;
  const uint8_t *packed = a.packed;
  const size_t in_stride = a.in_stride;
  const uint32_t *sizes = a.sizes;
  const RegionArgs &ra = a.ra;
  const TensK td = &((const __attribute__((address_space(4))) RegionArgsT *)__builtin_amdgcn_kernarg_segment_ptr())->t;
#include "dec_body_region.inc"
}

struct RegionArgsP {
  Geom g;
  DecWs ws;
  const uint8_t *packed;
  size_t in_stride;
  const uint32_t *sizes;
  RegionArgs ra;
  DstDesc d;
};
__global__ __launch_bounds__(kDecThreads) void k_dec_region_p(RegionArgsP a) {
  constexpr bool kRegionTens = false, kRegionPitch = true;
  const Geom &g = a.g;
  const DecWs &ws = a.ws;
  const uint8_t *packed = a.packed;
  const size_t in_stride = a.in_stride;
  const uint32_t *sizes = a.sizes;
  const RegionArgs &ra = a.ra;
  const TensK td = nullptr;
  const DstK pd = &((const __attribute__((address_space(4))) RegionArgsP *)__builtin_amdgcn_kernarg_segment_ptr())->d;
#include "dec_body_region.inc"
}

__device__ __forceinline__ int region_r0(const int32_t *org, int f) { return org[2 * f + 1] / 8; }
__device__ __forceinline__ int region_r1(const int32_t *org, int f, int h) { return (org[2 * f + 1] + h + 7) / 8; }

__global__ __launch_bounds__(64) void k_region_rowwalk(Geom g, DecWs ws, const uint8_t *packed, size_t in_stride,
                                                       const uint32_t *sizes, const int32_t *org, int h) {
  const int r1_f = region_r1(org, blockIdx.x, h);
  const int row_end = r1_f == g.rows ? 0x7fffffff : r1_f, resume = 0;
#include "dec_body_rowwalk.inc"
}

__global__ __launch_bounds__(256) void k_region_set_index(Geom g, DecWs ws_all, const uint32_t *index_all,
                                                          const uint32_t *sizes_all, const int32_t *org, int h) {
  const int f_ = blockIdx.x;
  DecWs ws = ws_all;
  ws.frames += f_;
  ws.row_off += (size_t)f_ * g.rows;
  ws.row_len += (size_t)f_ * g.rows;
  const uint32_t *index = index_all + (size_t)f_ * 2 * g.rows, *sizes = sizes_all + f_;
  const int r0 = region_r0(org, f_), r1 = region_r1(org, f_, h);
#include "dec_body_set_index.inc"
}

__global__ __launch_bounds__(kDecThreads, 8) void k_region_count(Geom g, DecWs ws, const uint8_t *packed,
                                                                size_t in_stride, const uint32_t *sizes,
                                                                const int32_t *org, int h, int rows_per_wg) {
  constexpr bool LDSPAY = false;
  const int r0 = region_r0(org, blockIdx.y), r1 = region_r1(org, blockIdx.y, h);
  if (r0 + (int)blockIdx.x * rows_per_wg >= r1) return;
#include "dec_body_row_count.inc"
}

__global__ __launch_bounds__(kDecThreads, 8) void k_region_count_w(Geom g, DecWs ws, const uint8_t *packed,
                                                                  size_t in_stride, const uint32_t *sizes,
                                                                  const int32_t *org, int h) {
  const int r0 = region_r0(org, blockIdx.y), r1 = region_r1(org, blockIdx.y, h);
  if (r0 + (int)blockIdx.x * kCountRowsW >= r1) return;
#include "dec_body_row_count_w.inc"
}

__global__ void k_region_walk_end(Geom g, DecWs ws, const uint8_t *packed, size_t in_stride, const int32_t *org, int h,
                                  int batch) {
  const int f = blockIdx.x * blockDim.x + threadIdx.x;
  if (f >= batch) return;
  const int r1 = region_r1(org, f, h);
  if (r1 >= g.rows) return;
  DecFrame *df = ws.frames + f;
  if (df->parse_status != 0 || df->walk_status != fmt_err(7, 1) || df->walk_q != 0) return;
  const uint8_t *p = packed + (size_t)f * in_stride;
  const uint32_t end = df->s[1].chunk_end;
  uint32_t q = df->s[1].payload_off;
  for (int r = 0; r < r1; ++r) {
    if (q + 2 > end) return;
    uint32_t len = p[q] | (p[q + 1] << 8);
    q += 2;
    if (len & 0x8000u) {
      if (q + 2 > end) return;
      len = (len & 0x7fffu) | ((uint32_t)(p[q] | (p[q + 1] << 8)) << 15);
      q += 2;
    }
    if (len > end - q) return;
    q += len;
  }
  if (q == end) df->walk_status = 0;
}

constexpr int kStShort = 5;

__global__ __launch_bounds__(64) void k_prefix_gate(Geom g, DecWs ws, const uint8_t *packed, size_t in_stride,
                                                    const uint32_t *avails, uint32_t *ptx, uint32_t *pbound,
                                                    int32_t *krows, int32_t *gate) {
  __shared__ uint8_t s_tree[kTreeStride];
  __shared__ uint32_t s_hdr[4];
  const int f = blockIdx.x, lane = threadIdx.x;
  DecFrame *df = ws.frames + f;
  const uint8_t *p = packed + (size_t)f * in_stride;
  const uint32_t avail = avails[f];
  if (lane == 0) {
    PfxHead h;
    int rc = pfx_chain(p, avail, g.fix_t2, (uint32_t)g.row_block, &h);
    const bool geom = h.frmt && ((int)h.W != g.W || (int)h.H != g.H || (int)h.C != g.C);
    if (geom) rc = kPfxFormat;
    if (rc == kPfxFormat && !geom && h.need > avail) rc = kPfxShort;
    s_hdr[0] = (uint32_t)rc; s_hdr[1] = h.coff; s_hdr[2] = h.csz; s_hdr[3] = h.T;
    df->walk_status = rc == kPfxFormat ? (geom ? kStGeom : fmt_err(h.stage, h.huff)) : 0;
    df->rows_first = 0;
    df->walk_q = 0;
    krows[f] = 0;
  }
  __syncthreads();
  int rc = (int)s_hdr[0];
  const uint32_t coff = s_hdr[1], csz = s_hdr[2], T = s_hdr[3];
  uint32_t have = 0;
  if (rc == kPfxOk) {
    const uint32_t cnt = csz < (uint32_t)kTreeStride ? csz : (uint32_t)kTreeStride;
    have = avail > coff ? (avail - coff < cnt ? avail - coff : cnt) : 0u;
    for (uint32_t k = lane; k < have; k += 64u) s_tree[k] = p[coff + k];
  }
  __syncthreads();
  if (lane != 0) return;
  if (rc == kPfxOk) {
    uint32_t tb = 0;
    rc = pfx_tree_len(s_tree, have, csz, &tb);
    if (rc == kPfxFormat) {
      df->walk_status = fmt_err(7, 1);
    } else if (rc == kPfxOk) {
      const uint32_t q = coff + tb, end = coff + csz;
      if (q < end) { df->rows_first = q; df->walk_q = q; df->walk_end = end; }
    }
  }
  const bool is_short = rc == kPfxShort;
  gate[f] = is_short ? kStShort : 0;
  ptx[f] = is_short ? 0u : T;
  pbound[f] = is_short ? 0u : avail;
}

__global__ __launch_bounds__(64) void k_prefix_rowwalk(Geom g, DecWs ws, const uint8_t *packed, size_t in_stride,
                                                       const uint32_t *pbound, const uint32_t *ptx, int32_t *krows,
                                                       int batch) {
  const int f = blockIdx.x * 64 + threadIdx.x;
  if (f >= batch) return;
  DecFrame *df = ws.frames + f;
  const uint32_t q = df->walk_q;
  if (q == 0) return;
  df->walk_q = 0;
  PfxRows pr;
  const int rc = pfx_rows(packed + (size_t)f * in_stride, pbound[f], ptx[f], g.fix_t2, g.rows, q, df->walk_end,
                          ws.row_off + (size_t)f * g.rows, ws.row_len + (size_t)f * g.rows, &pr);
  if (rc == kPfxFormat) { df->walk_status = fmt_err(7, 1); return; }
  krows[f] = pr.k;
}

__global__ __launch_bounds__(kDecThreads, 8) void k_prefix_count(Geom g, DecWs ws, const uint8_t *packed,
                                                                size_t in_stride, const uint32_t *sizes,
                                                                const int32_t *krows, int rows_per_wg) {
  constexpr bool LDSPAY = false;
  const int r0 = 0, r1 = krows[blockIdx.y];
  if ((int)blockIdx.x * rows_per_wg >= r1) return;
#include "dec_body_row_count.inc"
}

__global__ __launch_bounds__(kDecThreads, 8) void k_prefix_count_w(Geom g, DecWs ws, const uint8_t *packed,
                                                                  size_t in_stride, const uint32_t *sizes,
                                                                  const int32_t *krows) {
  const int r0 = 0, r1 = krows[blockIdx.y];
  if ((int)blockIdx.x * kCountRowsW >= r1) return;
#include "dec_body_row_count_w.inc"
}

struct PrefixArgs {
  const int32_t *krows;
  int sw;
  uint8_t *out;
};
struct PrefixOrigin {
  __device__ __forceinline__ int operator[](int) const { return 0; }
};
struct PrefixWindow {
  PrefixOrigin org;
  int sw, w, h;
  uint8_t *out;
};
__global__ __launch_bounds__(kDecThreads) void k_dec_prefix(Geom g, DecWs ws, const uint8_t *packed, size_t in_stride,
                                                           const uint32_t *sizes, PrefixArgs pa) {
  constexpr bool kRegionTens = false, kRegionPitch = false;
  const TensK td = nullptr;
  const DstK pd = nullptr;
  const int k_f = pa.krows[blockIdx.z];
  if ((int)blockIdx.y >= k_f) return;
  PrefixWindow ra;
  ra.sw = pa.sw; ra.w = g.W; ra.h = 8 * k_f < g.H ? 8 * k_f : g.H;
  ra.out = pa.out + (size_t)blockIdx.z * ((size_t)(g.H - ra.h) * g.W * g.C);
#include "dec_body_region.inc"
}

__device__ __forceinline__ void fill_half(uint32_t l4, uint32_t r4, int hh, uint32_t x[4]) {
  const uint32_t rnd = 0x01010101u;
  const uint32_t m4 = __builtin_amdgcn_lerp(l4, r4, rnd);
  const uint32_t lo = hh ? m4 : l4, hi = hh ? r4 : m4;
  const uint32_t m = __builtin_amdgcn_lerp(lo, hi, rnd);
  x[0] = lo; x[1] = __builtin_amdgcn_lerp(lo, m, rnd); x[2] = m; x[3] = __builtin_amdgcn_lerp(m, hi, rnd);
}

__global__ __launch_bounds__(256) void k_prefix_fill(Geom g, DecWs ws, const int32_t *krows, uint8_t *out) {
  const int f = blockIdx.z, v = blockIdx.y;
  if (v < krows[f]) return;
  const DecFrame *df = ws.frames + f;
  if (df->status != 0 || (df->parse_status == 0 && df->walk_status != 0)) return;
  const int it = (int)blockIdx.x * 256 + (int)threadIdx.x, u = it >> 1, hh = it & 1;
  const int cols = g.cols, C = g.C, W = g.W, H = g.H;
  if (u >= cols) return;
  const int v2 = v + 1 < g.rows ? v + 1 : g.rows - 1, u2 = u + 1 < cols ? u + 1 : cols - 1;
  const uint8_t *low = ws.low + (size_t)f * ws.plane_stride;
  uint32_t X[4][2][4];
#pragma unroll
  for (int c = 0; c < 4; ++c) {
    if (c < C) {
      const uint8_t *m = low + (size_t)c * g.rows * cols;
      uint32_t lr[9];
      lr[0] = (uint32_t)m[(size_t)v * cols + u] | ((uint32_t)m[(size_t)v * cols + u2] << 8);
      lr[8] = (uint32_t)m[(size_t)v2 * cols + u] | ((uint32_t)m[(size_t)v2 * cols + u2] << 8);
      interp9_u8x4(lr);
#pragma unroll
      for (int q = 0; q < 2; ++q) {
        const uint32_t p01 = __builtin_amdgcn_perm(lr[4 * q + 1], lr[4 * q], 0x05010400u);
        const uint32_t p23 = __builtin_amdgcn_perm(lr[4 * q + 3], lr[4 * q + 2], 0x05010400u);
        fill_half(__builtin_amdgcn_perm(p23, p01, 0x05040100u), __builtin_amdgcn_perm(p23, p01, 0x07060302u), hh,
                  X[c][q]);
      }
    } else {
#pragma unroll
      for (int q = 0; q < 2; ++q)
#pragma unroll
        for (int k = 0; k < 4; ++k) X[c][q][k] = 0;
    }
  }
  const int ycc = df->ycbcr;
  const int x0 = 8 * u + 4 * hh, y0 = 8 * v;
  if (x0 >= W) return;
  uint8_t *img = out + (size_t)f * ((size_t)H * W * C);
  const bool wide = C == 4 && x0 + 4 <= W && ((((uintptr_t)img) | ((size_t)W * 4)) & 15u) == 0;
#pragma unroll
  for (int q = 0; q < 2; ++q) {
#pragma unroll
    for (int i = 0; i < 4; ++i) {
      const int y = y0 + 4 * q + i;
      if (y >= H) continue;
      uint32_t px[4];
#pragma unroll
// ... 546 lines not shown
  }
  hipError_t e = hipFuncSetAttribute(reinterpret_cast<const void *>(&k_row_window), hipFuncAttributeMaxDynamicSharedMemorySize,
                                     (int)kRowWindowLds);
  if (e != hipSuccess) return e;
  hipFuncAttributes fa;
  e = hipFuncGetAttributes(&fa, reinterpret_cast<const void *>(&k_dec_region));
  if (e == hipSuccess)
    e = hipFuncSetAttribute(reinterpret_cast<const void *>(&k_dec_region), hipFuncAttributeMaxDynamicSharedMemorySize,
                            (int)(kLdsMax - fa.sharedSizeBytes));
  if (e == hipSuccess) e = hipFuncGetAttributes(&fa, reinterpret_cast<const void *>(&k_dec_region_t));
  if (e == hipSuccess)
    e = hipFuncSetAttribute(reinterpret_cast<const void *>(&k_dec_region_t), hipFuncAttributeMaxDynamicSharedMemorySize,
                            (int)(kLdsMax - fa.sharedSizeBytes));
  if (e == hipSuccess) e = hipFuncGetAttributes(&fa, reinterpret_cast<const void *>(&k_dec_region_p));
  if (e == hipSuccess)
    e = hipFuncSetAttribute(reinterpret_cast<const void *>(&k_dec_region_p), hipFuncAttributeMaxDynamicSharedMemorySize,
                            (int)(kLdsMax - fa.sharedSizeBytes));
  if (e == hipSuccess) e = hipFuncGetAttributes(&fa, reinterpret_cast<const void *>(&k_dec_prefix));
  if (e == hipSuccess)
    e = hipFuncSetAttribute(reinterpret_cast<const void *>(&k_dec_prefix), hipFuncAttributeMaxDynamicSharedMemorySize,
                            (int)(kLdsMax - fa.sharedSizeBytes));
  const void *scaled[] = {reinterpret_cast<const void *>(&k_dec_scaled<4, true>), reinterpret_cast<const void *>(&k_dec_scaled<2, true>),
                          reinterpret_cast<const void *>(&k_dec_scaled<4, false>), reinterpret_cast<const void *>(&k_dec_scaled<2, false>),
                          reinterpret_cast<const void *>(&k_dec_scaled_region<4>), reinterpret_cast<const void *>(&k_dec_scaled_region<2>)};
  for (const void *k : scaled) {
    if (e == hipSuccess) e = hipFuncGetAttributes(&fa, k);
    if (e == hipSuccess)
      e = hipFuncSetAttribute(k, hipFuncAttributeMaxDynamicSharedMemorySize, (int)(kLdsMax - fa.sharedSizeBytes));
  }
  return e;
}

int region_strip_tiles(const Geom &g) {
  const uint32_t fixed = region_layout(g.C, 0).total - region_layout(g.C, 0).seg * 64u * (uint32_t)g.C;
  const uint32_t seg = (kLdsMax - 1024u - fixed) / (64u * (uint32_t)g.C) & ~3u;
  return (int)(seg - 8u);
}

int scaled_strip_tiles(const Geom &g, int scale_log2) {
  const uint32_t nseg = (scale_log2 == 1 ? 16u : 4u) * (uint32_t)g.C;
  const RegionLayout L0 = scale_log2 == 1 ? scaled_layout<4>(g.C, 0) : scaled_layout<2>(g.C, 0);
  const uint32_t fixed = L0.total - L0.seg * nseg;
  const uint32_t seg = (kLdsMax - 1024u - fixed) / nseg & ~3u;
  return (int)(seg - 8u);
}

void launch_rowwalk_only(const Geom &g, const DecWs &ws, const uint8_t *d_packed, size_t in_stride,
                         const uint32_t *d_sizes, hipStream_t stream) {
  hipLaunchKernelGGL(k_dec_rowwalk, dim3(1), dim3(64), 0, stream, g, ws, d_packed, in_stride, d_sizes, 0x7fffffff, 0);
}

void launch_rowwalk_range(const Geom &g, const DecWs &ws, const uint8_t *d_packed, size_t in_stride,
                          const uint32_t *d_sizes, int row_end, bool resume, hipStream_t stream) {
  hipLaunchKernelGGL(k_dec_rowwalk, dim3(1), dim3(64), 0, stream, g, ws, d_packed, in_stride, d_sizes, row_end, resume ? 1 : 0);
}

static void launch_lres_chain(const Geom &g, const DecWs &ws, int batch, const uint8_t *d_packed, size_t in_stride,
                              const uint32_t *d_sizes, hipStream_t stream, Profiler *prof) {
  HIMG_LAUNCH(k_lres_spec, dim3(ws.lres_chunks, batch), dim3(kDecThreads), g, ws, d_packed, in_stride, d_sizes);
  HIMG_LAUNCH(k_lres_fix, dim3(batch), dim3(kDecThreads), g, ws, d_packed, in_stride, d_sizes);
  HIMG_LAUNCH(k_lres_write, dim3(ws.lres_chunks, batch), dim3(kDecThreads), g, ws, d_packed,
              in_stride, d_sizes);
  HIMG_LAUNCH(k_lres_finish, dim3((batch + 63) / 64), dim3(64), ws, batch);
  HIMG_LAUNCH(k_lres_unpredict, dim3((g.mcols + 4 * kUnpredWaves - 1) / (4 * kUnpredWaves), g.mrows, batch * g.C),
              dim3(64 * kUnpredWaves), g, ws);
}

static void launch_zero(const Geom &g, const DecWs &ws, int batch, hipStream_t stream, Profiler *prof) {
  const uint32_t n16 = (uint32_t)(((size_t)batch * ws.lres_stride + 15) / 16);
  const uint32_t ns = (uint32_t)((size_t)batch * (g.rows + 1) * 8), nr = ws.rc_stats ? (uint32_t)((size_t)batch * g.rows * 8) : 0u;
  prof_begin(prof, "memset", stream);
  hipLaunchKernelGGL(k_dec_zero, dim3((n16 + 256 * 4 - 1) / (256 * 4)), dim3(256), 0, stream,
                     reinterpret_cast<uint4 *>(ws.lres_sym), n16, ws.stats, ns, ws.rc_stats, nr);
  prof_end(prof, stream);
}

struct CountRule { bool wave; int rpc; Geom g; };
static CountRule count_rule(const Geom &g, long long all_rows, bool one_record) {
  CountRule c = {g.count_wave >= 0 ? g.count_wave != 0 : all_rows >= 8192,
                 all_rows <= 512 ? 1 : all_rows <= 1024 ? 2 : kRowsPerCount, g};
  if (one_record) c.g.max_sub = 0x7fffffff;
  return c;
}

void launch_preview(const Geom &g, const DecWs &ws, int batch, const uint8_t *d_packed, size_t in_stride,
                    const uint32_t *d_sizes, uint32_t *d_head_sizes, uint8_t *d_out, int32_t *d_status,
                    hipStream_t stream, Profiler *prof) {
  launch_zero(g, ws, batch, stream, prof);
  HIMG_LAUNCH(k_dec_parse_head, dim3(batch), dim3(kParseThreads), g, ws, d_packed, in_stride, d_sizes, d_head_sizes);
  launch_lres_chain(g, ws, batch, d_packed, in_stride, d_head_sizes, stream, prof);
  const uint32_t npix = (uint32_t)g.rows * (uint32_t)g.cols;
  HIMG_LAUNCH(k_lres_preview, dim3((npix + 1023u) / 1024u, batch), dim3(256), g, ws, d_out);
  HIMG_LAUNCH(k_dec_status, dim3((batch + 63) / 64), dim3(64), ws, d_status, batch);
}

struct WindowExtents { int nrows = 0, ntiles = 0; long long all_rows = 0; bool stop_early = false; };
static WindowExtents window_extents(const Geom &g, int batch, const int32_t *h_org, int S, int w, int h) {
  WindowExtents e;
  const int F = 8 / S;
  for (int f = 0; f < batch; ++f) {
    const int x = h_org[2 * f] / F, y = h_org[2 * f + 1] / F;
    const int r0 = y / S, r1 = (y + h + S - 1) / S, nt = (x + w + S - 1) / S - x / S;
    e.nrows = r1 - r0 > e.nrows ? r1 - r0 : e.nrows;
    e.ntiles = nt > e.ntiles ? nt : e.ntiles;
    e.stop_early |= r1 < g.rows;
    e.all_rows += r1 - r0;
  }
  return e;
}

void launch_region(const Geom &g, const DecWs &ws_in, int batch, const uint8_t *d_packed, size_t in_stride,
                   const uint32_t *d_sizes, const uint32_t *d_row_index, const int32_t *h_org, const int32_t *d_org,
                   int scale_log2, int w, int h, uint8_t *d_out, int32_t *d_status, hipStream_t stream, Profiler *prof,
                   const DecStreams *ds, const TensDesc *tens, const DstDesc *dst) {
  DecWs ws = ws_in;
  ws.lane_q = nullptr;
  const int F = 1 << scale_log2, hf = F * h;
  const WindowExtents e = window_extents(g, batch, h_org, 8 / F, w, h);
  launch_zero(g, ws, batch, stream, prof);
  hipStream_t ws_ = ds ? ds->side : stream;
  if (ds) {
    (void)hipEventRecord(ds->ev_fork, stream);
    (void)hipStreamWaitEvent(ws_, ds->ev_fork, 0);
  }
  prof_begin(prof, d_row_index ? "k_region_set_index" : "k_region_rowwalk", ws_);
  if (d_row_index)
    hipLaunchKernelGGL(k_region_set_index, dim3(batch), dim3(256), 0, ws_, g, ws, d_row_index, d_sizes, d_org, hf);
  else
    hipLaunchKernelGGL(k_region_rowwalk, dim3(batch), dim3(64), 0, ws_, g, ws, d_packed, in_stride, d_sizes, d_org, hf);
  prof_end(prof, ws_);
  if (ds) (void)hipEventRecord(ds->ev_walk[0], ws_);
  HIMG_LAUNCH(k_dec_parse, dim3(batch), dim3(kParseThreads), g, ws, d_packed, in_stride, d_sizes);
  launch_lres_chain(g, ws, batch, d_packed, in_stride, d_sizes, stream, prof);
  if (ds) (void)hipStreamWaitEvent(stream, ds->ev_walk[0], 0);
  if (!d_row_index && e.stop_early)
    HIMG_LAUNCH(k_region_walk_end, dim3((batch + 63) / 64), dim3(64), g, ws, d_packed, in_stride, d_org, hf, batch);
  const CountRule cr = count_rule(g, e.all_rows, true);
  if (cr.wave) {
    HIMG_LAUNCH(k_region_count_w, dim3((e.nrows + kCountRowsW - 1) / kCountRowsW, batch), dim3(kDecThreads), cr.g, ws,
                d_packed, in_stride, d_sizes, d_org, hf);
  } else {
    HIMG_LAUNCH(k_region_count, dim3((e.nrows + cr.rpc - 1) / cr.rpc, batch), dim3(kDecThreads), cr.g, ws, d_packed,
                in_stride, d_sizes, d_org, hf, cr.rpc);
  }
  const int smax = scale_log2 ? scaled_strip_tiles(g, scale_log2) : region_strip_tiles(g);
  const int nstrip = (e.ntiles + smax - 1) / smax, sw = (e.ntiles + nstrip - 1) / nstrip;
  const dim3 grid(nstrip, e.nrows, batch);
  if (!scale_log2) {
    RegionArgs ra;
    ra.org = d_org; ra.sw = sw; ra.w = w; ra.h = h; ra.out = d_out;
    prof_begin(prof, tens ? "k_dec_region_t" : dst ? "k_dec_region_p" : "k_dec_region", stream);
    if (dst) {
      RegionArgsP rp;
      rp.g = g; rp.ws = ws; rp.packed = d_packed; rp.in_stride = in_stride; rp.sizes = d_sizes; rp.ra = ra; rp.d = *dst;
      hipLaunchKernelGGL(k_dec_region_p, grid, dim3(kDecThreads), region_layout(g.C, sw).total, stream, rp);
    } else if (tens) {
      RegionArgsT rt;
      rt.g = g; rt.ws = ws; rt.packed = d_packed; rt.in_stride = in_stride; rt.sizes = d_sizes; rt.ra = ra; rt.t = *tens;
      hipLaunchKernelGGL(k_dec_region_t, grid, dim3(kDecThreads), region_layout(g.C, sw).total, stream, rt);
    } else
    hipLaunchKernelGGL(k_dec_region, grid, dim3(kDecThreads), region_layout(g.C, sw).total, stream, g, ws, d_packed,
                       in_stride, d_sizes, ra);
  } else {
    ScaledRegionArgs sa;
    sa.org = d_org; sa.sw = sw; sa.w = w; sa.h = h; sa.out = d_out;
    prof_begin(prof, "k_dec_scaled_region", stream);
    if (scale_log2 == 1)
      hipLaunchKernelGGL(k_dec_scaled_region<4>, grid, dim3(kDecThreads), scaled_layout<4>(g.C, sw).total, stream, g, ws,
                         d_packed, in_stride, d_sizes, sa);
    else
      hipLaunchKernelGGL(k_dec_scaled_region<2>, grid, dim3(kDecThreads), scaled_layout<2>(g.C, sw).total, stream, g, ws,
                         d_packed, in_stride, d_sizes, sa);
  }
  prof_end(prof, stream);
  HIMG_LAUNCH(k_dec_status, dim3((batch + 63) / 64), dim3(64), ws, d_status, batch);
}

void launch_prefix(const Geom &g, const DecWs &ws_in, int batch, const uint8_t *d_packed, size_t in_stride,
                   uint32_t *d_words, uint8_t *d_out, int32_t *d_rows, int32_t *d_status, hipStream_t stream,
                   Profiler *prof, const DecStreams *ds) {
  DecWs ws = ws_in;
  ws.lane_q = nullptr;
  const uint32_t *d_avail = d_words;
  uint32_t *d_tx = d_words + batch, *d_bound = d_words + 2 * (size_t)batch;
  int32_t *d_k = (int32_t *)(d_words + 3 * (size_t)batch), *d_gate = (int32_t *)(d_words + 4 * (size_t)batch);
  launch_zero(g, ws, batch, stream, prof);
  HIMG_LAUNCH(k_prefix_gate, dim3(batch), dim3(64), g, ws, d_packed, in_stride, d_avail, d_tx, d_bound, d_k, d_gate);
  hipStream_t ws_ = ds ? ds->side : stream;
  if (ds) {
    (void)hipEventRecord(ds->ev_fork, stream);
    (void)hipStreamWaitEvent(ws_, ds->ev_fork, 0);
  }
  prof_begin(prof, "k_prefix_rowwalk", ws_);
  hipLaunchKernelGGL(k_prefix_rowwalk, dim3((batch + 63) / 64), dim3(64), 0, ws_, g, ws, d_packed, in_stride, d_bound, d_tx,
                     d_k, batch);
  prof_end(prof, ws_);
  if (ds) (void)hipEventRecord(ds->ev_walk[0], ws_);
  HIMG_LAUNCH(k_dec_parse_prefix, dim3(batch), dim3(kParseThreads), g, ws, d_packed, in_stride, d_tx, d_bound);
  launch_lres_chain(g, ws, batch, d_packed, in_stride, d_bound, stream, prof);
  if (ds) (void)hipStreamWaitEvent(stream, ds->ev_walk[0], 0);
  HIMG_LAUNCH(k_prefix_fill, dim3((2 * g.cols + 255) / 256, g.rows, batch), dim3(256), g, ws, d_k, d_out);
  const CountRule cr = count_rule(g, (long long)batch * g.rows, true);
  if (cr.wave) {
    HIMG_LAUNCH(k_prefix_count_w, dim3((g.rows + kCountRowsW - 1) / kCountRowsW, batch), dim3(kDecThreads), cr.g, ws,
                d_packed, in_stride, d_bound, d_k);
  } else {
    HIMG_LAUNCH(k_prefix_count, dim3((g.rows + cr.rpc - 1) / cr.rpc, batch), dim3(kDecThreads), cr.g, ws, d_packed,
                in_stride, d_bound, d_k, cr.rpc);
  }
  const int smax = region_strip_tiles(g);
  const int nstrip = (g.cols + smax - 1) / smax, sw = (g.cols + nstrip - 1) / nstrip;
  PrefixArgs pa;
  pa.krows = d_k; pa.sw = sw; pa.out = d_out;
  prof_begin(prof, "k_dec_prefix", stream);
  hipLaunchKernelGGL(k_dec_prefix, dim3(nstrip, g.rows, batch), dim3(kDecThreads), region_layout(g.C, sw).total, stream, g,
                     ws, d_packed, in_stride, d_bound, pa);
  prof_end(prof, stream);
  HIMG_LAUNCH(k_prefix_status, dim3((batch + 63) / 64), dim3(64), ws, d_gate, d_k, d_status, d_rows, batch);
}

void launch_scaled(const Geom &g, const DecWs &ws_in, int batch, const uint8_t *d_packed, size_t in_stride,
                   const uint32_t *d_sizes, const uint32_t *d_row_index, int scale_log2, uint8_t *d_out,
                   int32_t *d_status, hipStream_t stream, Profiler *prof, const DecStreams *ds) {
  constexpr int kWalkAll = 0x7fffffff;
  DecWs ws = ws_in;
  ws.lane_q = nullptr;
  const int F = 1 << scale_log2;
  launch_zero(g, ws, batch, stream, prof);
  hipStream_t side = ds ? ds->side : stream;
  auto walk = [&](hipStream_t s) {
    prof_begin(prof, d_row_index ? "k_dec_set_index" : "k_dec_rowwalk", s);
    if (d_row_index)
      hipLaunchKernelGGL(k_dec_set_index, dim3(1), dim3(256), 0, s, g, ws, d_row_index, d_sizes, 0, g.rows);
    else
      hipLaunchKernelGGL(k_dec_rowwalk, dim3(batch), dim3(64), 0, s, g, ws, d_packed, in_stride, d_sizes, kWalkAll, 0);
    prof_end(prof, s);
  };
  const CountRule cr = count_rule(g, (long long)batch * g.rows, true);
  auto row_count = [&](hipStream_t s) {
    prof_begin(prof, "k_row_count", s);
    if (cr.wave)
      hipLaunchKernelGGL(k_row_count_w, dim3((g.rows + kCountRowsW - 1) / kCountRowsW, batch), dim3(kDecThreads), 0, s, cr.g,
                         ws, d_packed, in_stride, d_sizes, 0, g.rows);
    else
      hipLaunchKernelGGL(k_row_count<false>, dim3((g.rows + cr.rpc - 1) / cr.rpc, batch), dim3(kDecThreads), 0, s, cr.g, ws,
                         d_packed, in_stride, d_sizes, 0, g.rows, cr.rpc);
    prof_end(prof, s);
  };
  if (ds) {
    (void)hipEventRecord(ds->ev_fork, stream);
    (void)hipStreamWaitEvent(side, ds->ev_fork, 0);
    walk(side);
  }
  HIMG_LAUNCH(k_dec_parse, dim3(batch), dim3(kParseThreads), g, ws, d_packed, in_stride, d_sizes);
  if (ds) {
    (void)hipEventRecord(ds->ev_fork, stream);
    (void)hipStreamWaitEvent(side, ds->ev_fork, 0);
    row_count(side);
    (void)hipEventRecord(ds->ev_cnt[0], side);
  } else {
    walk(stream);
  }
  launch_lres_chain(g, ws, batch, d_packed, in_stride, d_sizes, stream, prof);
  if (ds) (void)hipStreamWaitEvent(stream, ds->ev_cnt[0], 0);
  else row_count(stream);
  ScaledArgs sa;
  const uint32_t lds_one = scale_log2 == 1 ? scaled_layout_one<4>(g.C, g.cols).total : scaled_layout_one<2>(g.C, g.cols).total;
  const bool one = lds_one <= kLdsMax - 1024u;
  const int smax = scaled_strip_tiles(g, scale_log2), nstrip = one ? 1 : (g.cols + smax - 1) / smax;
  sa.sw = (g.cols + nstrip - 1) / nstrip;
  sa.ow = (g.W + F - 1) / F; sa.oh = (g.H + F - 1) / F; sa.out = d_out;
  prof_begin(prof, "k_dec_scaled", stream);
#define HIMG_SCALED_LAUNCH(S_, ONE_, LDS_)                                                                        \
  hipLaunchKernelGGL((k_dec_scaled<S_, ONE_>), dim3(nstrip, g.rows, batch), dim3(kDecThreads), LDS_, stream, g, ws, \
                     d_packed, in_stride, d_sizes, sa)
  if (scale_log2 == 1 && one) HIMG_SCALED_LAUNCH(4, true, lds_one);
  else if (scale_log2 == 1) HIMG_SCALED_LAUNCH(4, false, scaled_layout<4>(g.C, sa.sw).total);
  else if (one) HIMG_SCALED_LAUNCH(2, true, lds_one);
  else HIMG_SCALED_LAUNCH(2, false, scaled_layout<2>(g.C, sa.sw).total);
#undef HIMG_SCALED_LAUNCH
  prof_end(prof, stream);
  HIMG_LAUNCH(k_dec_status, dim3((batch + 63) / 64), dim3(64), ws, d_status, batch);
}

void launch_decode(const Geom &g, const DecWs &ws, int batch, const uint8_t *d_packed,
                   size_t in_stride, const uint32_t *d_sizes, uint8_t *d_out,
                   int32_t *d_status, hipStream_t stream, Profiler *prof, const HostOpts &ho,
                   const DecStreams *ds, int r0, int r1,
                   const uint32_t *d_row_index, bool index_only, int phase, const TensDesc *tens,
                   const DstDesc *dst, const PyrDesc *pyr) {
  constexpr int kWalkAll = 0x7fffffff;
  const bool do_head = (phase & kDecHead) != 0, do_rows = (phase & kDecRows) != 0;
  if (index_only) {
    HIMG_LAUNCH(k_dec_parse, dim3(batch), dim3(kParseThreads), g, ws, d_packed, in_stride, d_sizes);
    HIMG_LAUNCH(k_dec_rowwalk, dim3(batch), dim3(64), g, ws, d_packed, in_stride, d_sizes, r1 == 0 ? 0 : kWalkAll, 0);
    HIMG_LAUNCH(k_dec_status, dim3((batch + 63) / 64), dim3(64), ws, d_status, batch);
    return;
  }
  const int nrows = r1 - r0;
  const CountRule cr = count_rule(g, (long long)batch * nrows, false);
  const unsigned gx = (unsigned)((((g.cols + 31) / 32) * 64 + 255) / 256);
  const int wps = (ho.allow_fused && fused_layout(g.row_block).total <= kLdsMax) ? 1 : 0;
  const int seg_env = ho.walk_segs;
  const int seg_want = seg_env ? (seg_env < 1 ? 1 : seg_env > kWalkSegs ? kWalkSegs : seg_env)
                               : (nrows >= 1024 ? (wps ? 2 : kWalkSegs) : 1);
  const int nseg = (ds && batch == 1 && !d_row_index && r0 == 0 && r1 == g.rows && nrows >= 16 * kWalkSegs) ? seg_want : 1;
  hipStream_t side = ds ? ds->side : nullptr;
  hipStream_t cnt_stream = !ds ? stream : nseg > 1 ? ds->side2 : ds->side;
  auto seg_lo = [&](int k) { return r0 + (int)((long long)nrows * k / nseg); };
  if (do_head) launch_zero(g, ws, batch, stream, prof);
  if (ds && do_rows) {
    (void)hipEventRecord(ds->ev_fork, stream);
    (void)hipStreamWaitEvent(side, ds->ev_fork, 0);
    if (d_row_index) {
      prof_begin(prof, "k_dec_set_index", side);
      hipLaunchKernelGGL(k_dec_set_index, dim3(1), dim3(256), 0, side, g, ws, d_row_index, d_sizes, r0, r1);
      prof_end(prof, side);
      (void)hipEventRecord(ds->ev_walk[0], side);
    } else {
      for (int k = 0; k < nseg; ++k) {
        prof_begin(prof, "k_dec_rowwalk", side);
        hipLaunchKernelGGL(k_dec_rowwalk, dim3(batch), dim3(64), 0, side, g, ws, d_packed, in_stride, d_sizes,
                           k + 1 < nseg ? seg_lo(k + 1) : kWalkAll, k > 0 ? 1 : 0);
        prof_end(prof, side);
        (void)hipEventRecord(ds->ev_walk[k], side);
      }
    }
  }
  if (do_head) HIMG_LAUNCH(k_dec_parse, dim3(batch), dim3(kParseThreads), g, ws, d_packed, in_stride, d_sizes);
  auto row_count = [&](hipStream_t s, int a, int b) {
    if (b <= a) return;
    prof_begin(prof, "k_row_count", s);
    if (cr.wave)
      hipLaunchKernelGGL(k_row_count_w, dim3((b - a + kCountRowsW - 1) / kCountRowsW, batch), dim3(kDecThreads), 0, s,
                         g, ws, d_packed, in_stride, d_sizes, a, b);
    else if (wps)
      hipLaunchKernelGGL(k_row_count<true>, dim3((b - a + cr.rpc - 1) / cr.rpc, batch), dim3(kDecThreads), 0, s, g, ws,
                         d_packed, in_stride, d_sizes, a, b, cr.rpc);
    else if (ws.lane_q && g.wide_q && g.count_wave < 0 && (g.row_block % 16) == 0)
      hipLaunchKernelGGL(k_row_count_q, dim3(b - a, batch), dim3(kDecThreads), 0, s, g, ws, d_packed, in_stride, d_sizes, a);
    else
      hipLaunchKernelGGL(k_row_count<false>, dim3((b - a + cr.rpc - 1) / cr.rpc, batch), dim3(kDecThreads), 0, s, g, ws,
                         d_packed, in_stride, d_sizes, a, b, cr.rpc);
    prof_end(prof, s);
  };
  const bool window = (g.row_block % 16) == 0;
  auto window_pass = [&](hipStream_t s, int a, int b) {
    if (b <= a) return;
    if (window) {
      const unsigned nwin = (unsigned)(((uint32_t)g.row_block + kRowWindow - 1u) / kRowWindow);
      prof_begin(prof, "k_row_window", s);
      hipLaunchKernelGGL(k_row_window, dim3(nwin, b - a, batch), dim3(kDecThreads), kRowWindowLds, s, g, ws, d_packed,
                         in_stride, d_sizes, a);
      prof_end(prof, s);
    }
    prof_begin(prof, "k_dec_huff", s);
    hipLaunchKernelGGL(k_dec_huff, dim3(b - a, batch), dim3(kDecThreads), 0, s, g, ws, d_packed, in_stride,
                       d_sizes, 1 + a, 1, window ? 2 : 1);
    prof_end(prof, s);
  };
  if (!do_rows) {
  } else if (ds) {
    (void)hipEventRecord(ds->ev_fork, stream);
    (void)hipStreamWaitEvent(cnt_stream, ds->ev_fork, 0);
    for (int k = 0; k < nseg; ++k) {
      if (cnt_stream != side) (void)hipStreamWaitEvent(cnt_stream, ds->ev_walk[k], 0);
      row_count(cnt_stream, seg_lo(k), seg_lo(k + 1));
      (void)hipEventRecord(ds->ev_cnt[k], cnt_stream);
      if (!wps) {
        hipStream_t ws_ = (nseg > 1 && ds->side3) ? ds->side3 : cnt_stream;
        if (ws_ != cnt_stream) (void)hipStreamWaitEvent(ws_, ds->ev_cnt[k], 0);
        window_pass(ws_, seg_lo(k), seg_lo(k + 1));
        (void)hipEventRecord(ds->ev_win[k], ws_);
      }
    }
  } else if (d_row_index) {
    HIMG_LAUNCH(k_dec_set_index, dim3(1), dim3(256), g, ws, d_row_index, d_sizes, r0, r1);
  } else {
    HIMG_LAUNCH(k_dec_rowwalk, dim3(batch), dim3(64), g, ws, d_packed, in_stride, d_sizes, kWalkAll, 0);
  }
  if (do_head) launch_lres_chain(g, ws, batch, d_packed, in_stride, d_sizes, stream, prof);
  if (do_head && pyr && pyr->level[3]) {
    const uint32_t npix = (uint32_t)g.rows * (uint32_t)g.cols;
    HIMG_LAUNCH(k_lres_preview, dim3((npix + 1023u) / 1024u, batch), dim3(256), g, ws, pyr->level[3]);
  }
  if (!do_rows) return;
  if (wps) {
    const int per_row = ((g.cols + 31) / 32) * 64;
    int rpw = 1;
    while (rpw < 8 && (rpw + 1) * per_row <= kDecThreads && fused_layout(g.row_block, rpw + 1).total <= kLdsMax) ++rpw;
    if (g.W == 4096 && g.C == 4 && (g.H & 7) == 0) rpw = 1;
    const uint32_t lds = fused_layout(g.row_block, rpw).total;
    const int n_cu = ho.n_cu, per_cu = 1;
#define HIMG_FUSED_LAUNCH(COLS, A, B)                                                           \
  do {                                                                                          \
    const int gx_ = ((B) - (A) + rpw - 1) / rpw;                                                \
    const long long all_ = (long long)gx_ * batch;                                              \
    const int slots_ = ho.persist_rows > 1 ? ho.persist_rows : n_cu * per_cu;                   \
    const bool pers_ = ho.persist_rows != 0 && all_ > slots_;                                   \
    RowArgs ra_;                                                                                \
    ra_.g = g; ra_.ws = ws; ra_.packed = d_packed; ra_.in_stride = in_stride; ra_.sizes = d_sizes; \
    ra_.out_frames = d_out; ra_.r0 = (A); ra_.r1 = (B); ra_.rpw = rpw; ra_.gx = gx_; ra_.gy = batch; \
    ra_.next_dist = pers_ ? 0 : n_cu * per_cu;                                                 \
    if (tens) {                                                                                 \
      RowArgsT rt_;                                                                             \
      rt_.a = ra_; rt_.t = *tens;                                                               \
      hipLaunchKernelGGL((k_dec_row_fused_t<(COLS) == 256 || (COLS) == 240 ? -1 : (COLS)>),     \
                         dim3((unsigned)(pers_ ? slots_ : all_)), dim3(kDecThreads), lds, stream, rt_); \
    } else if (dst) {                                                                           \
      RowArgsP rp_;                                                                             \
      rp_.a = ra_; rp_.d = *dst;                                                                \
      hipLaunchKernelGGL((k_dec_row_fused_p<(COLS) == 256 || (COLS) == 240 ? -1 : (COLS)>),     \
                         dim3((unsigned)(pers_ ? slots_ : all_)), dim3(kDecThreads), lds, stream, rp_); \
    } else if (pyr) {                                                                           \
      RowArgsM rm_;                                                                             \
      rm_.a = ra_; rm_.m = *pyr;                                                                \
      hipLaunchKernelGGL((k_dec_row_fused_m<(COLS) == 256 || (COLS) == 240 ? -1 : (COLS)>),     \
                         dim3((unsigned)(pers_ ? slots_ : all_)), dim3(kDecThreads), lds, stream, rm_); \
// ... 99 lines not shown
```

include/himg_hip.h:

```cpp
#ifndef HIMG_HIP_H_
#define HIMG_HIP_H_

#include <stddef.h>
#include <stdint.h>

#ifdef __cplusplus
extern "C" {
#endif

#define HIMG_OK 0
#define HIMG_ERR_ARG (-1)
#define HIMG_ERR_HIP (-2)
#define HIMG_ERR_UNSUPPORTED (-3)
#define HIMG_ERR_FORMAT (-4)
#define HIMG_ERR_CAPACITY (-5)
#define HIMG_ERR_TARGET (-6)

typedef struct himg_hip_ctx himg_hip_ctx;

int himg_hip_create(int device, himg_hip_ctx **ctx);
void himg_hip_destroy(himg_hip_ctx *ctx);
const char *himg_hip_last_error(const himg_hip_ctx *ctx);

#define HIMG_OPT_FIX_T2 1
#define HIMG_OPT_COUNT_WAVE 2
#define HIMG_OPT_EMIT_ROWS 3
#define HIMG_OPT_ROW_TOKENS 4
#define HIMG_OPT_FRONT 5
int himg_hip_set_option(himg_hip_ctx *ctx, int option, int value);
int himg_hip_get_option(himg_hip_ctx *ctx, int option, int *value);

size_t himg_hip_max_packed_size(int width, int height, int num_channels);


int himg_hip_encode(himg_hip_ctx *ctx, const uint8_t *data, int width, int height,
                    int pixel_stride, int num_channels, int quality, int use_ycbcr,
                    uint8_t **out, size_t *out_size);

int himg_hip_decode(himg_hip_ctx *ctx, const uint8_t *packed, size_t packed_size,
                    uint8_t **out, int *width, int *height, int *num_channels);

void himg_hip_free(void *p);

int himg_hip_encode_to(himg_hip_ctx *ctx, const uint8_t *data, int width, int height,
                       int pixel_stride, int num_channels, int quality, int use_ycbcr,
                       uint8_t *dst, size_t dst_cap, size_t *out_size);
int himg_hip_decode_to(himg_hip_ctx *ctx, const uint8_t *packed, size_t packed_size, uint8_t *dst,
                       size_t dst_cap, int *width, int *height, int *num_channels);
int himg_hip_fetch_last(himg_hip_ctx *ctx, uint8_t *dst, size_t dst_cap, size_t *size);
int himg_hip_peek(const uint8_t *packed, size_t packed_size, int *width, int *height,
                  int *num_channels);

int himg_hip_encode_batch(himg_hip_ctx *ctx, const uint8_t *const *frames, int n, int width,
                          int height, int pixel_stride, int num_channels, int quality,
                          int use_ycbcr, uint8_t *const *dst, const size_t *dst_cap,
                          size_t *out_sizes);
int himg_hip_decode_batch(himg_hip_ctx *ctx, const uint8_t *const *packed, const size_t *packed_sizes,
                          int n, uint8_t *const *dst, const size_t *dst_cap, int *widths,
                          int *heights, int *channels);

void *himg_hip_host_alloc(size_t bytes);
void himg_hip_host_free(void *p);


int himg_hip_encode_device(himg_hip_ctx *ctx, const void *d_frames, int batch,
                           int width, int height, int pixel_stride,
                           int num_channels, int quality, int use_ycbcr,
                           void *d_out, size_t out_stride, uint32_t *d_sizes,
                           int32_t *d_status, void *stream);

int himg_hip_decode_device(himg_hip_ctx *ctx, const void *d_packed, size_t in_stride,
                           const uint32_t *h_sizes, int batch, int width, int height,
                           int num_channels, void *d_out, int32_t *d_status,
                           void *stream);

int himg_hip_encode_device_q(himg_hip_ctx *ctx, const void *d_frames, int batch, int width, int height,
                             int pixel_stride, int num_channels, const int32_t *h_quality, int use_ycbcr,
                             void *d_out, size_t out_stride, uint32_t *d_sizes, int32_t *d_status,
                             void *stream);
int himg_hip_encode_sizes_device(himg_hip_ctx *ctx, const void *d_frames, int batch, int width, int height,
                                 int pixel_stride, int num_channels, const int32_t *h_quality,
                                 int use_ycbcr, uint32_t *d_sizes, int32_t *d_status, void *stream);
int himg_hip_budget_probes(int qmin, int qmax);
int himg_hip_encode_budget_device(himg_hip_ctx *ctx, const void *d_frames, int batch, int width, int height,
                                  int pixel_stride, int num_channels, int qmin, int qmax, int use_ycbcr,
                                  const uint32_t *h_budgets, void *d_out, size_t out_stride,
                                  uint32_t *d_sizes, int32_t *d_quality, int32_t *d_status, void *stream);
int himg_hip_encode_budget_to(himg_hip_ctx *ctx, const uint8_t *data, int width, int height,
                              int pixel_stride, int num_channels, int qmin, int qmax, int use_ycbcr,
                              size_t budget, uint8_t *dst, size_t dst_cap, size_t *out_size, int *quality);
int himg_hip_encode_budget_batch(himg_hip_ctx *ctx, const uint8_t *const *frames, int n, int width,
                                 int height, int pixel_stride, int num_channels, int qmin, int qmax,
                                 int use_ycbcr, const size_t *budgets, uint8_t *const *dst,
                                 const size_t *dst_cap, size_t *out_sizes, int *qualities);

typedef struct himg_hip_src {
  int width, height;
  int pixel_stride;
  size_t row_pitch;
  size_t frame_pitch;
} himg_hip_src;

int himg_hip_windows_extent(const himg_hip_src *src, int num_channels, int batch,
                            const int32_t *h_origins, int w, int h, size_t *bytes);
int himg_hip_encode_windows_device(himg_hip_ctx *ctx, const void *d_src, const himg_hip_src *src,
                                   int batch, int num_channels, const int32_t *h_origins, int w, int h,
                                   const int32_t *h_quality, int use_ycbcr, void *d_out, size_t out_stride,
                                   uint32_t *d_sizes, int32_t *d_status, void *stream);
int himg_hip_encode_window_to(himg_hip_ctx *ctx, const uint8_t *data, const himg_hip_src *src,
                              int num_channels, int x, int y, int w, int h, int quality, int use_ycbcr,
                              uint8_t *dst, size_t dst_cap, size_t *out_size);
// ... 157 lines not shown
                            const uint32_t *d_all_row_bits, const void *d_rel, size_t rel_bytes,
                            void *d_out, size_t out_cap, uint32_t *d_size, int32_t *d_status,
                            void *stream);
int himg_hip_shard_head(himg_hip_ctx *ctx, const uint8_t *d_low_full, const uint32_t *d_all_row_bits,
                        void *d_out, size_t out_cap, uint32_t *d_size, uint32_t *d_head,
                        int32_t *d_status, void *stream);
int himg_hip_shard_finish(himg_hip_ctx *ctx, void *d_out, size_t out_cap, const uint32_t *d_size,
                          void *stream);

int himg_hip_decode_rows_device(himg_hip_ctx *ctx, const void *d_packed, uint32_t packed_size,
                                int width, int height, int num_channels, int row0, int row1,
                                void *d_out_rows, int32_t *d_status, void *stream);

int himg_hip_decode_index_device(himg_hip_ctx *ctx, const void *d_packed, uint32_t packed_size,
                                 int width, int height, int num_channels, uint32_t *d_row_index,
                                 uint32_t *d_rows_first, int32_t *d_status, void *stream);
int himg_hip_index_host(const uint8_t *packed, size_t packed_size, int fix_t2, int *width, int *height,
                        int *num_channels, uint32_t *row_index, size_t index_rows,
                        uint32_t *rows_first);
int himg_hip_decode_rows_indexed_device(himg_hip_ctx *ctx, const void *d_packed, uint32_t packed_size,
                                        int width, int height, int num_channels, int row0, int row1,
                                        const uint32_t *d_row_index, void *d_out_rows,
                                        int32_t *d_status, void *stream);
int himg_hip_decode_head_device(himg_hip_ctx *ctx, const void *d_packed, uint32_t packed_size,
                                int width, int height, int num_channels, void *stream);
int himg_hip_decode_rows_after_head_device(himg_hip_ctx *ctx, const void *d_packed, uint32_t packed_size,
                                           int width, int height, int num_channels, int row0, int row1,
                                           const uint32_t *d_row_index, void *d_out_rows,
                                           int32_t *d_status, void *stream);
int himg_hip_decode_first_device(himg_hip_ctx *ctx, const void *d_packed, uint32_t packed_size,
                                 int width, int height, int num_channels, uint32_t *d_rows_first,
                                 int32_t *d_status, void *stream);
int himg_hip_decode_walk_device(himg_hip_ctx *ctx, const void *d_packed, uint32_t packed_size,
                                int width, int height, int num_channels, uint32_t *d_row_index,
                                uint32_t *d_rows_first, int32_t *d_status, void *stream);
int himg_hip_decode_walk_wait(himg_hip_ctx *ctx);
#define HIMG_MAX_WALK_RANGES 16
int himg_hip_decode_walk_ranges_device(himg_hip_ctx *ctx, const void *d_packed, uint32_t packed_size,
                                       int width, int height, int num_channels, const int *range_end,
                                       int n_ranges, uint32_t *d_row_index, uint32_t *d_rows_first,
                                       int32_t *d_range_status, void *stream);
int himg_hip_decode_walk_wait_range(himg_hip_ctx *ctx, int k);

typedef struct himg_hip_multi himg_hip_multi;
int himg_hip_create_multi(const int *devices, int n, himg_hip_multi **out);
void himg_hip_destroy_multi(himg_hip_multi *m);
int himg_hip_multi_count(const himg_hip_multi *m);
const char *himg_hip_multi_last_error(const himg_hip_multi *m);
int himg_hip_multi_set_option(himg_hip_multi *m, int option, int value);
int himg_hip_multi_encode_batch(himg_hip_multi *m, const uint8_t *const *frames, int n, int width,
                                int height, int pixel_stride, int num_channels, int quality,
                                int use_ycbcr, uint8_t *const *dst, const size_t *dst_cap,
                                size_t *out_sizes);
int himg_hip_multi_decode_batch(himg_hip_multi *m, const uint8_t *const *packed,
                                const size_t *packed_sizes, int n, uint8_t *const *dst,
                                const size_t *dst_cap, int *widths, int *heights, int *channels);
int himg_hip_multi_encode(himg_hip_multi *m, const uint8_t *data, int width, int height,
                          int pixel_stride, int num_channels, int quality, int use_ycbcr,
                          uint8_t **out, size_t *out_size);
int himg_hip_multi_decode(himg_hip_multi *m, const uint8_t *packed, size_t packed_size, uint8_t **out,
                          int *width, int *height, int *num_channels);


enum {
  HIMG_DBG_AVG = 0,
  HIMG_DBG_LOWRES = 1,
  HIMG_DBG_LRES_SYM = 2,
  HIMG_DBG_FRES_SYM = 3,
  HIMG_DBG_LRES_HIST = 4,
  HIMG_DBG_FRES_HIST = 5,
  HIMG_DBG_LRES_LEN = 6,
  HIMG_DBG_FRES_LEN = 7,
  HIMG_DBG_LRES_CODE = 8,
  HIMG_DBG_FRES_CODE = 9,
  HIMG_DBG_FRES_ROW_BYTES = 10,
  HIMG_DBG_DEC_STATS = 11,
  HIMG_DBG_PARSE_STATS = 12,
  HIMG_DBG_ROWCOUNT_STATS = 13,
  HIMG_DBG_LOOP_COUNTS = 14
  ,
  HIMG_DBG_FRES_TOK_SYM = 15
  ,
  HIMG_DBG_TOK_CNT = 16
};
int himg_hip_debug_read(himg_hip_ctx *ctx, int what, int frame, void *host_dst,
                        size_t dst_bytes, size_t *bytes_written);

#define HIMG_MAX_STAGES 32
int himg_hip_profile_enable(himg_hip_ctx *ctx, int enable);
int himg_hip_profile_reset(himg_hip_ctx *ctx);
int himg_hip_profile_read(himg_hip_ctx *ctx, int *n_stages,
                          const char *names[HIMG_MAX_STAGES],
                          double ms[HIMG_MAX_STAGES], int launches[HIMG_MAX_STAGES]);


int himg_hip_tok_layout(int width, int height, int pixel_stride, int num_channels, int row_tokens, int batch,
                        int out[6]);

enum { HIMG_SYNTH_GRAD = 0, HIMG_SYNTH_GRADN = 1, HIMG_SYNTH_RAND = 2, HIMG_SYNTH_RANDTILE = 3 };
int himg_synth_fill(int kind, uint64_t seed, int width, int height, uint8_t *rgba);
uint64_t himg_fnv1a64(const uint8_t *data, size_t n);

void himg_tables_shift(int quality, int chroma, uint8_t out[64]);
void himg_tables_lowres_map(int quality, int16_t out[128]);
void himg_tables_fullres_map(int16_t out[128]);
uint8_t himg_tables_map_to_8bit(const int16_t table[128], int x);

#ifdef __cplusplus
}
#endif
#endif
```

Baseline: 99370.

## Have each lane of the wave row-count kernel walk several consecutive sub-sequences

The wavefront row-count kernel gains a stretch mode in which each lane handles NQ consecutive sub-sequences (four by default) instead of one. Each lane stages its own small slice of the bitstream into LDS and runs the self-synchronising count across its stretch, stopping early when it rejoins a previously found boundary. Per-sub-sequence start and offset records are then scattered through LDS. The intent is fewer fix-up rounds and less wave-level synchronisation per row, at the cost of more serial work per lane and a different LDS staging layout. Debug entry points and an option for choosing the stretch factor are also added.

```diff
diff --git a/himg_amd/__init__.py b/himg_amd/__init__.py
--- a/himg_amd/__init__.py
+++ b/himg_amd/__init__.py
@@ -23,6 +23,7 @@
     "avg": 0, "lowres": 1, "lres_sym": 2, "fres_sym": 3, "lres_hist": 4, "fres_hist": 5,
     "lres_len": 6, "fres_len": 7, "lres_code": 8, "fres_code": 9, "fres_row_bytes": 10,
     "dec_stats": 11, "parse_stats": 12, "rowcount_stats": 13, "loop_counts": 14, "fres_tok_sym": 15, "tok_cnt": 16,
+    "lane_start": 17, "lane_off": 18,
 }
 DBG_DECODER = 0x100
 
@@ -75,6 +76,7 @@
     L.himg_hip_host_free.restype = None
     L.himg_hip_encode_device.argtypes = [vp, vp, i32, i32, i32, i32, i32, i32, i32, vp, sz, vp, vp, vp]
     L.himg_hip_decode_device.argtypes = [vp, vp, sz, vp, i32, i32, i32, i32, vp, vp, vp]
+    L.himg_hip_debug_row_records.argtypes = [vp, vp, sz, vp, i32, i32, i32, i32, vp, vp]
     L.himg_hip_encode_device_q.argtypes = [vp, vp, i32, i32, i32, i32, i32, vp, i32, vp, sz, vp, vp, vp]
     L.himg_hip_windows_extent.argtypes = [vp, i32, i32, vp, i32, i32, P(sz)]
     L.himg_hip_encode_windows_device.argtypes = [vp, vp, vp, i32, i32, vp, i32, i32, vp, i32, vp, sz, vp, vp, vp]
@@ -224,7 +226,7 @@
 
 
 
-_OPTIONS = {"fix_t2": 1, "count_wave": 2, "emit_rows": 3, "row_tokens": 4, "front": 5}
+_OPTIONS = {"fix_t2": 1, "count_wave": 2, "emit_rows": 3, "row_tokens": 4, "front": 5, "count_stretch": 6}
 
 
 class Engine:
@@ -675,6 +677,12 @@
                                           _ptr(d_status), C.c_void_p(stream))
         self._check(rc, "decode_device")
 
+    def row_records_device(self, d_packed, in_stride, h_sizes, batch, width, height, channels, d_status, stream=0):
+        hs = np.ascontiguousarray(h_sizes, np.uint32)
+        rc = lib().himg_hip_debug_row_records(self._ctx, _ptr(d_packed), in_stride, hs.ctypes.data,
+                                              batch, width, height, channels, _ptr(d_status), C.c_void_p(stream))
+        self._check(rc, "row_records_device")
+
     def decode_tensor_device(self, d_packed, in_stride, h_sizes, batch, width, height, channels, desc, d_out,
                              d_status, stream=0):
         hs = np.ascontiguousarray(h_sizes, np.uint32)
diff --git a/himg_amd/csrc/dec_body_row_count_w.inc b/himg_amd/csrc/dec_body_row_count_w.inc
--- a/himg_amd/csrc/dec_body_row_count_w.inc
+++ b/himg_amd/csrc/dec_body_row_count_w.inc
@@ -1,6 +1,6 @@
   __shared__ __attribute__((aligned(16))) uint32_t gyx[2 * kTabEntries];
   __shared__ uint32_t nd[kMaxNodes + 1];
-  __shared__ __attribute__((aligned(16))) uint32_t s_stage[kCountRowsW * kStageAlloc];
+  __shared__ __attribute__((aligned(16))) uint32_t s_stage[kCountRowsW * (NQ > 1 ? kLaneAlloc : kStageAlloc)];
   __shared__ int s_flag;
   uint32_t *gy = gyx, *gx = gyx + kTabEntries;
   const int f = blockIdx.y, tid = threadIdx.x, lane = tid & 63;
@@ -52,7 +52,7 @@
   uint32_t first = rel0;
   uint32_t base = 0;
   uint32_t rounds = 0;
-  uint32_t *stage = s_stage + (tid >> 6) * kStageAlloc;
+  uint32_t *stage = s_stage + (tid >> 6) * (NQ > 1 ? kLaneAlloc : kStageAlloc);
   LdsBits bits;
   bits.base = lds_addr(stage);
   auto phases = [&](auto staged_c) {
@@ -139,8 +139,152 @@
     first = (uint32_t)__builtin_amdgcn_readlane((int)(active ? endpos + shift : rel_end), 63);
   }
   };
-  if (sb <= kStageSubBits) phases(std::true_type{});
-  else phases(std::false_type{});
+  auto stretches = [&]() {
+    uint32_t *piece = stage + (uint32_t)lane * kLaneWords;
+    LaneBits lb;
+    lb.base = 0;
+    auto stage_at = [&](uint32_t pos, bool on) {
+      wave_lds_sync();
+      if (on) {
+        const uint32_t w0 = pos >> 5;
+        if (w0 + kLaneWords - 1u <= rd.jmax) {
+#pragma unroll
+          for (uint32_t i = 0; i + 4u <= kLaneWords; i += 4u) {
+            const PackedU4 u = *reinterpret_cast<const PackedU4 *>(rd.w + w0 + i);
+            piece[i] = u.x; piece[i + 1u] = u.y; piece[i + 2u] = u.z; piece[i + 3u] = u.w;
+          }
+#pragma unroll
+          for (uint32_t i = kLaneWords & ~3u; i < kLaneWords; ++i) piece[i] = rd.w[w0 + i];
+        } else {
+#pragma unroll 1
+          for (uint32_t i = 0; i < kLaneWords; ++i) piece[i] = rd.ld(w0 + i);
+        }
+        lb.base = lds_addr(piece) - 4u * w0;
+      }
+      wave_lds_sync();
+    };
+    const uint32_t la = (rem - 1u) / sb, L = rem - la * sb;
+    const uint32_t S = (L > kTailBits && la + 1u < (uint32_t)kDecThreads) ? sb - (L - kTailBits) : 0u;
+    const uint32_t last_active = (rem - 1u + S) / sb;
+    auto nom_b0 = [&](uint32_t v) { return v ? rel0 + v * sb - S : rel0; };
+    auto nom_lim = [&](uint32_t v) { const uint32_t x = rel0 + (v + 1u) * sb - S; return x > rel_end ? rel_end : x; };
+    const uint32_t lead_in = lead < 256u ? lead : 256u;
+#pragma unroll 1
+    for (int j = 0; j < kDecThreads / (64 * NQ); ++j) {
+      const uint32_t v0 = (uint32_t)(64 * j + lane) * (uint32_t)NQ;
+      const uint32_t b0 = nom_b0(v0);
+      uint32_t *t_start = l_start + 64 * NQ * j + lane, *t_off = l_off + 64 * NQ * j + lane;
+      const bool active = b0 < rel_end;
+      const uint32_t pb0 = (uint32_t)__builtin_amdgcn_readfirstlane((int)b0);
+      if (pb0 >= rel_end) {
+#pragma unroll
+        for (int k = 0; k < NQ; ++k) { t_start[64 * k] = rem; t_off[64 * k] = base; }
+        continue;
+      }
+      uint32_t start = active ? b0 : rel_end;
+      if (lane == 0) start = first;
+      if (lead_in) {
+        const bool on = lane > 0 && active;
+        const uint32_t from = start - rel0 > lead_in ? start - lead_in : rel0;
+        stage_at(from, on);
+        if (on) {
+          uint32_t guess, none;
+          grp_count_lds(lb, tb, from, start, &guess, &none);
+          start = guess;
+        }
+      }
+      uint32_t endpos = start, cnt0 = 0;
+      bool dirty = active;
+      uint32_t T = b0 + kJoinBits;
+      { const uint32_t lim0 = nom_lim(v0); if (T > lim0 || T < b0) T = lim0; }
+      uint32_t posT = ~0u, cT = 0;
+      bool again = false;
+      for (;;) {
+        bool walking = dirty;
+        uint32_t pos = start;
+#pragma unroll 1
+        for (int k = 0; k < NQ; ++k) {
+          if (!__any(walking ? 1 : 0)) break;
+          const uint32_t lim = nom_lim(v0 + (uint32_t)k);
+          stage_at(pos, walking);
+          if (walking) {
+            uint32_t np = pos, c;
+            if (k == 0) {
+              uint32_t p1, c1;
+              grp_count_lds(lb, tb, pos, T, &p1, &c1);
+              if (p1 == posT) {
+                c = c1 + (cnt0 - cT);
+                walking = false;
+              } else {
+                uint32_t c2;
+                grp_count_lds(lb, tb, p1, lim, &np, &c2);
+                c = c1 + c2;
+              }
+              posT = p1;
+              cT = c1;
+              cnt0 = c;
+            } else {
+              grp_count_lds(lb, tb, pos, lim, &np, &c);
+            }
+            t_off[64 * k] = c;
+            if (walking) {
+              if (k + 1 < NQ) {
+                uint32_t *m = t_start + 64 * (k + 1);
+                if (again && *m == np - rel0) walking = false;
+                else *m = np - rel0;
+              } else {
+                endpos = np;
+              }
+              pos = np;
+            }
+          }
+        }
+        const uint32_t ns = wave_shr1_dpp(first, endpos);
+        dirty = active && ns != start;
+        if (active) start = ns;
+        ++rounds;
+        again = true;
+        if (!__any(dirty ? 1 : 0)) break;
+      }
+      uint32_t tot = 0;
+      if (active) {
+#pragma unroll
+        for (int k = 0; k < NQ; ++k) tot += min(t_off[64 * k], 0x3fffffu);
+      }
+      const uint32_t incl = wave_scan_add_dpp(tot);
+      wave_lds_sync();
+#pragma unroll
+      for (int k = 0; k < NQ; ++k) {
+        const uint32_t v = v0 + (uint32_t)k;
+        const bool a = nom_b0(v) < rel_end;
+        if (v == last_active) l_off[kDecThreads + 1] = k + 1 < NQ ? t_start[64 * (k + 1)] : endpos - rel0;
+        stage[(uint32_t)lane * NQ + k] = k == 0 ? start - rel0 : (a ? t_start[64 * k] : rem);
+      }
+      wave_lds_sync();
+#pragma unroll
+      for (int k = 0; k < NQ; ++k) t_start[64 * k] = stage[64 * k + lane];
+      wave_lds_sync();
+      uint32_t off = base + incl - tot;
+#pragma unroll
+      for (int k = 0; k < NQ; ++k) {
+        const bool a = nom_b0(v0 + (uint32_t)k) < rel_end;
+        stage[(uint32_t)lane * NQ + k] = off;
+        off += a ? min(t_off[64 * k], 0x3fffffu) : 0u;
+      }
+      wave_lds_sync();
+#pragma unroll
+      for (int k = 0; k < NQ; ++k) t_off[64 * k] = stage[64 * k + lane];
+      base += (uint32_t)__builtin_amdgcn_readlane((int)incl, 63);
+      first = (uint32_t)__builtin_amdgcn_readlane((int)(active ? endpos : rel_end), 63);
+    }
+  };
+  if constexpr (NQ > 1) {
+    if (sb <= kStageSubBits) stretches();
+    else phases(std::false_type{});
+  } else {
+    if (sb <= kStageSubBits) phases(std::true_type{});
+    else phases(std::false_type{});
+  }
   if (lane == 0) {
     l_off[kDecThreads] = base;
     l_off[kDecThreads + 3] = rounds;
diff --git a/himg_amd/csrc/himg_dev.h b/himg_amd/csrc/himg_dev.h
--- a/himg_amd/csrc/himg_dev.h
+++ b/himg_amd/csrc/himg_dev.h
@@ -30,6 +30,7 @@
   int lead_bits;
   int prefetch_rows;
   int count_wave;
+  int count_stretch;
   int wide_q;
   int emit_rows;
   int front;
@@ -276,6 +277,8 @@
                    const uint32_t *d_row_index = nullptr, bool index_only = false, int phase = 3,
                    const TensDesc *tens = nullptr, const DstDesc *dst = nullptr, const PyrDesc *pyr = nullptr);
 constexpr int kDecHead = 1, kDecRows = 2;
+void launch_row_records(const Geom &g, const DecWs &ws, int batch, const uint8_t *d_packed, size_t in_stride,
+                        const uint32_t *d_sizes, int32_t *d_status, hipStream_t stream, Profiler *prof);
 void launch_preview(const Geom &g, const DecWs &ws, int batch, const uint8_t *d_packed, size_t in_stride,
                     const uint32_t *d_sizes, uint32_t *d_head_sizes, uint8_t *d_out, int32_t *d_status,
                     hipStream_t stream, Profiler *prof);
diff --git a/himg_amd/csrc/himg_hip.hip b/himg_amd/csrc/himg_hip.hip
--- a/himg_amd/csrc/himg_hip.hip
+++ b/himg_amd/csrc/himg_hip.hip
@@ -108,6 +108,7 @@
   int lres_serial = 0;
   int prefetch_rows = 1;
   int count_wave = -1, emit_rows = -1;
+  int count_stretch = -1;
   int row_tokens = -1;
   int front = -1;
   DecStreams dstr;
@@ -207,6 +208,7 @@
   g->lead_bits = 128;
   g->lres_serial = 0;
   g->count_wave = g->emit_rows = g->row_tokens = g->front = -1;
+  g->count_stretch = -1;
   g->wide_q = 0;
   g->prefetch_rows = 1;
   g->frame_bytes = (long long)width * height * pixel_stride;
@@ -221,6 +223,7 @@
   g->lres_serial = ctx->lres_serial;
   g->prefetch_rows = ctx->prefetch_rows;
   g->count_wave = ctx->count_wave;
+  g->count_stretch = ctx->count_stretch;
   g->emit_rows = ctx->emit_rows;
   g->row_tokens = ctx->row_tokens;
   g->front = ctx->front;
@@ -234,6 +237,8 @@
   n += (size_t)g.fres_size + kTreeStride + 4u * (size_t)g.rows;
   return round_up(n + 64, 256);
 }
+
+static bool stretch_ok(int v) { return v == -1 || v == 1 || v == 2 || v == 4 || v == 8; }
 
 extern "C" int himg_hip_create(int device, himg_hip_ctx **out) {
   if (!out) return HIMG_ERR_ARG;
@@ -257,6 +262,10 @@
     if (v >= 128 && v <= 4096 && v % 32 == 0) ctx->max_sub = v;
   }
   if (const char *e = std::getenv("HIMG_COUNT_WAVE")) ctx->count_wave = atoi(e) ? 1 : 0;
+  if (const char *e = std::getenv("HIMG_COUNT_STRETCH")) {
+    const int v = std::atoi(e);
+    if (stretch_ok(v)) ctx->count_stretch = v;
+  }
   if (const char *e = std::getenv("HIMG_EMIT_ROWS")) ctx->emit_rows = atoi(e) ? 1 : 0;
   if (const char *e = std::getenv("HIMG_ROW_TOKENS")) ctx->row_tokens = atoi(e) ? 1 : 0;
   if (const char *e = std::getenv("HIMG_FRONT")) ctx->front = atoi(e) ? 1 : 0;
@@ -362,12 +371,18 @@
   if (option == HIMG_OPT_EMIT_ROWS) { *value = ctx->emit_rows; return HIMG_OK; }
   if (option == HIMG_OPT_ROW_TOKENS) { *value = ctx->row_tokens; return HIMG_OK; }
   if (option == HIMG_OPT_FRONT) { *value = ctx->front; return HIMG_OK; }
+  if (option == HIMG_OPT_COUNT_STRETCH) { *value = ctx->count_stretch; return HIMG_OK; }
   return fail(ctx, HIMG_ERR_ARG, "unknown option");
 }
 
 extern "C" int himg_hip_set_option(himg_hip_ctx *ctx, int option, int value) {
   if (!ctx) return HIMG_ERR_ARG;
   if (option == HIMG_OPT_FIX_T2) { ctx->fix_t2 = value ? 1 : 0; return HIMG_OK; }
+  if (option == HIMG_OPT_COUNT_STRETCH) {
+    if (!stretch_ok(value)) return fail(ctx, HIMG_ERR_ARG, "count_stretch: -1, 1, 2, 4 or 8");
+    ctx->count_stretch = value;
+    return HIMG_OK;
+  }
   const int tri = value < 0 ? -1 : (value ? 1 : 0);
   if (option == HIMG_OPT_COUNT_WAVE) { ctx->count_wave = tri; return HIMG_OK; }
   if (option == HIMG_OPT_EMIT_ROWS) { ctx->emit_rows = tri; return HIMG_OK; }
@@ -996,6 +1011,22 @@
                      nullptr, nullptr, nullptr, nullptr);
 }
 
+extern "C" int himg_hip_debug_row_records(himg_hip_ctx *ctx, const void *d_packed, size_t in_stride,
+                                          const uint32_t *h_sizes, int batch, int width, int height,
+                                          int num_channels, int32_t *d_status, void *stream) {
+  if (!ctx || !d_packed || !h_sizes || !d_status || batch < 1 || batch > 65535) return HIMG_ERR_ARG;
+  Geom g;
+  const uint32_t *d_sizes = nullptr;
+  if (int rc = decode_args(ctx, width, height, num_channels, batch, kWsFull, d_packed, nullptr, &in_stride, nullptr, &g))
+    return rc;
+  if (int rc = stride_covers(ctx, h_sizes, batch, in_stride)) return rc;
+  if (int rc = decode_begin(ctx, g, batch, kWsFull, h_sizes, stream, &d_sizes)) return rc;
+  himg_dev::launch_row_records(g, ctx->dec_ws, batch, (const uint8_t *)d_packed, in_stride, d_sizes, d_status,
+                               (hipStream_t)stream, &ctx->prof);
+  HIP_TRY(ctx, hipGetLastError());
+  return HIMG_OK;
+}
+
 static bool tensor_desc_ok(const himg_hip_tensor_desc *t, int C, himg_dev::TensDesc *td) {
   if (!t || t->dtype < HIMG_DT_F32 || t->dtype > HIMG_DT_BF16 || t->out_channels < 1 || t->out_channels > C || C > 4)
     return false;
@@ -2726,6 +2757,10 @@
       case HIMG_DBG_FRES_SYM: src = w.fres_sym ? w.fres_sym + frame * w.fres_stride : nullptr; n = (size_t)g.fres_size; break;
       case HIMG_DBG_DEC_STATS: src = w.stats + (size_t)frame * (g.rows + 1) * 8; n = (size_t)(g.rows + 1) * 32; break;
       case HIMG_DBG_PARSE_STATS: src = w.parse_stats + (size_t)frame * 4; n = 16; break;
+      case HIMG_DBG_LANE_START: src = w.lane_start ? w.lane_start + (size_t)frame * g.rows * kDecThreads : nullptr; n = (size_t)g.rows * kDecThreads * 4; break;
+      case HIMG_DBG_LANE_OFF:
+        src = w.lane_off ? w.lane_off + (size_t)frame * g.rows * (kDecThreads + himg_dev::kRecHdr) : nullptr;
+        n = (size_t)g.rows * (kDecThreads + himg_dev::kRecHdr) * 4; break;
       case HIMG_DBG_ROWCOUNT_STATS: src = w.rc_stats ? w.rc_stats + (size_t)frame * g.rows * 8 : nullptr; n = (size_t)g.rows * 32; break;
       default: return HIMG_ERR_ARG;
     }
diff --git a/himg_amd/csrc/kernels_dec.hip b/himg_amd/csrc/kernels_dec.hip
--- a/himg_amd/csrc/kernels_dec.hip
+++ b/himg_amd/csrc/kernels_dec.hip
@@ -2945,6 +2945,16 @@
     return __builtin_amdgcn_alignbit(x.y, x.x, pos);
   }
 };
+constexpr uint32_t kLaneWords = 13;
+constexpr uint32_t kLaneAlloc = (64u * kLaneWords + 1u + 3u) & ~3u;
+struct LaneBits {
+  uint32_t base;
+  __device__ __forceinline__ uint32_t window(uint32_t pos) const {
+    const uint32_t a = base + ((pos >> 5) << 2);
+    const u32x2 x = *(const __attribute__((address_space(3))) u32x2_a4 *)(uintptr_t)a;
+    return __builtin_amdgcn_alignbit(x.y, x.x, pos);
+  }
+};
 constexpr uint32_t kStageSubBits = 320;
 constexpr uint32_t kStageWords = 64u * kStageSubBits / 32u + 32u;
 constexpr uint32_t kStageAlloc = (kStageWords + kStageWords / 32u + 3u) & ~3u;
@@ -2956,7 +2966,8 @@
   __device__ __forceinline__ void refill() {}
 };
 
-__device__ __forceinline__ void grp_count_lds(const LdsBits &bits, const GrpTables &t, uint32_t pos, uint32_t lim,
+template <class BITS>
+__device__ __forceinline__ void grp_count_lds(const BITS &bits, const GrpTables &t, uint32_t pos, uint32_t lim,
                                               uint32_t *endpos, uint32_t *count) {
   uint32_t c = 0;
   if (pos < lim) {
@@ -3001,11 +3012,21 @@
   *count = c;
 }
 
+constexpr int kCountStretch = 4;
 __global__ __launch_bounds__(kDecThreads, 8) void k_row_count_w(Geom g, DecWs ws, const uint8_t *packed,
                                                                size_t in_stride, const uint32_t *sizes,
                                                                int r0, int r1) {
+  constexpr int NQ = kCountStretch;
 #include "dec_body_row_count_w.inc"
 }
+template <int NQ>
+__global__ __launch_bounds__(kDecThreads, 8) void k_row_count_wn(Geom g, DecWs ws, const uint8_t *packed,
+                                                                size_t in_stride, const uint32_t *sizes,
+                                                                int r0, int r1) {
+#include "dec_body_row_count_w.inc"
+}
+static_assert((31u + kStageSubBits + 45u) / 32u < kLaneWords, "a sub-sequence and its overrun fit a lane's piece");
+static_assert(64 * 8 <= kLaneAlloc && 64 * kCountStretch <= kLaneAlloc, "a phase's 64 NQ records pass through a wavefront's staging buffer");
 
 constexpr int kQPhases = 4;
 __device__ __forceinline__ uint32_t *qrec_pos(uint32_t *l_start, uint32_t *l_q, uint32_t q) {
@@ -3658,6 +3679,7 @@
                                                                   const int32_t *org, int h) {
   const int r0 = region_r0(org, blockIdx.y), r1 = region_r1(org, blockIdx.y, h);
   if (r0 + (int)blockIdx.x * kCountRowsW >= r1) return;
+  constexpr int NQ = 1;
 #include "dec_body_row_count_w.inc"
 }
 
@@ -3767,6 +3789,7 @@
                                                                   const int32_t *krows) {
   const int r0 = 0, r1 = krows[blockIdx.y];
   if ((int)blockIdx.x * kCountRowsW >= r1) return;
+  constexpr int NQ = 1;
 #include "dec_body_row_count_w.inc"
 }
 
@@ -4479,6 +4502,18 @@
   if (one_record) c.g.max_sub = 0x7fffffff;
   return c;
 }
+static void launch_row_count_w(const Geom &g, const DecWs &ws, int batch, const uint8_t *d_packed, size_t in_stride,
+                               const uint32_t *d_sizes, int a, int b, hipStream_t s) {
+  const dim3 grid((b - a + kCountRowsW - 1) / kCountRowsW, batch), block(kDecThreads);
+  const int nq = g.count_stretch < 0 ? kCountStretch : g.count_stretch;
+#define HIMG_COUNT_WN(NQ_) hipLaunchKernelGGL(k_row_count_wn<NQ_>, grid, block, 0, s, g, ws, d_packed, in_stride, d_sizes, a, b)
+  if (nq == kCountStretch) hipLaunchKernelGGL(k_row_count_w, grid, block, 0, s, g, ws, d_packed, in_stride, d_sizes, a, b);
+  else if (nq == 2) HIMG_COUNT_WN(2);
+  else if (nq == 4) HIMG_COUNT_WN(4);
+  else if (nq == 8) HIMG_COUNT_WN(8);
+  else HIMG_COUNT_WN(1);
+#undef HIMG_COUNT_WN
+}
 
 void launch_preview(const Geom &g, const DecWs &ws, int batch, const uint8_t *d_packed, size_t in_stride,
                     const uint32_t *d_sizes, uint32_t *d_head_sizes, uint8_t *d_out, int32_t *d_status,
@@ -4637,8 +4672,7 @@
   auto row_count = [&](hipStream_t s) {
     prof_begin(prof, "k_row_count", s);
     if (cr.wave)
-      hipLaunchKernelGGL(k_row_count_w, dim3((g.rows + kCountRowsW - 1) / kCountRowsW, batch), dim3(kDecThreads), 0, s, cr.g,
-                         ws, d_packed, in_stride, d_sizes, 0, g.rows);
+      launch_row_count_w(cr.g, ws, batch, d_packed, in_stride, d_sizes, 0, g.rows, s);
     else
       hipLaunchKernelGGL(k_row_count<false>, dim3((g.rows + cr.rpc - 1) / cr.rpc, batch), dim3(kDecThreads), 0, s, cr.g, ws,
                          d_packed, in_stride, d_sizes, 0, g.rows, cr.rpc);
@@ -4676,6 +4710,17 @@
   else if (one) HIMG_SCALED_LAUNCH(2, true, lds_one);
   else HIMG_SCALED_LAUNCH(2, false, scaled_layout<2>(g.C, sa.sw).total);
 #undef HIMG_SCALED_LAUNCH
+  prof_end(prof, stream);
+  HIMG_LAUNCH(k_dec_status, dim3((batch + 63) / 64), dim3(64), ws, d_status, batch);
+}
+
+void launch_row_records(const Geom &g, const DecWs &ws, int batch, const uint8_t *d_packed, size_t in_stride,
+                        const uint32_t *d_sizes, int32_t *d_status, hipStream_t stream, Profiler *prof) {
+  launch_zero(g, ws, batch, stream, prof);
+  HIMG_LAUNCH(k_dec_parse, dim3(batch), dim3(kParseThreads), g, ws, d_packed, in_stride, d_sizes);
+  HIMG_LAUNCH(k_dec_rowwalk, dim3(batch), dim3(64), g, ws, d_packed, in_stride, d_sizes, 0x7fffffff, 0);
+  prof_begin(prof, "k_row_count", stream);
+  launch_row_count_w(g, ws, batch, d_packed, in_stride, d_sizes, 0, g.rows, stream);
   prof_end(prof, stream);
   HIMG_LAUNCH(k_dec_status, dim3((batch + 63) / 64), dim3(64), ws, d_status, batch);
 }
@@ -4729,8 +4774,7 @@
     if (b <= a) return;
     prof_begin(prof, "k_row_count", s);
     if (cr.wave)
-      hipLaunchKernelGGL(k_row_count_w, dim3((b - a + kCountRowsW - 1) / kCountRowsW, batch), dim3(kDecThreads), 0, s,
-                         g, ws, d_packed, in_stride, d_sizes, a, b);
+      launch_row_count_w(g, ws, batch, d_packed, in_stride, d_sizes, a, b, s);
     else if (wps)
       hipLaunchKernelGGL(k_row_count<true>, dim3((b - a + cr.rpc - 1) / cr.rpc, batch), dim3(kDecThreads), 0, s, g, ws,
                          d_packed, in_stride, d_sizes, a, b, cr.rpc);
diff --git a/include/himg_hip.h b/include/himg_hip.h
--- a/include/himg_hip.h
+++ b/include/himg_hip.h
@@ -27,6 +27,7 @@
 #define HIMG_OPT_EMIT_ROWS 3
 #define HIMG_OPT_ROW_TOKENS 4
 #define HIMG_OPT_FRONT 5
+#define HIMG_OPT_COUNT_STRETCH 6
 int himg_hip_set_option(himg_hip_ctx *ctx, int option, int value);
 int himg_hip_get_option(himg_hip_ctx *ctx, int option, int *value);
 
@@ -350,9 +351,16 @@
   HIMG_DBG_FRES_TOK_SYM = 15
   ,
   HIMG_DBG_TOK_CNT = 16
+  ,
+  HIMG_DBG_LANE_START = 17,
+  HIMG_DBG_LANE_OFF = 18
 };
 int himg_hip_debug_read(himg_hip_ctx *ctx, int what, int frame, void *host_dst,
                         size_t dst_bytes, size_t *bytes_written);
+
+int himg_hip_debug_row_records(himg_hip_ctx *ctx, const void *d_packed, size_t in_stride,
+                               const uint32_t *h_sizes, int batch, int width, int height,
+                               int num_channels, int32_t *d_status, void *stream);
 
 #define HIMG_MAX_STAGES 32
 int himg_hip_profile_enable(himg_hip_ctx *ctx, int enable);
```

Measured after the change: 101,400 (median of 6 runs). +2.1%, better.
